# fpthink/PDGN

Measured on AMD Instinct MI355X. Metric: generator+D step points/sec (B=35, 256->2048 pts), higher is better.
Workload: dtype f32; 1 GPU; PDGNet_v2 G+D iteration (models/PDGNet_v2.py:171-256), chair-shaped synthetic batch, per-GPU batch 35, 256->2048 pts, random-init weights; global_batch=35, parallelism=dp1, losses_finite=True, hipgraph=False, issue=list

## Files before the change

include/pdgn_hip.h:

```cpp
#ifndef PDGN_HIP_H
#define PDGN_HIP_H

#include <stdint.h>

#ifdef __cplusplus
extern "C" {
#endif

#define PDGN_ERR_INVALID (-1)
#define PDGN_KNN_MAX_NSAMPLE 200

typedef void *pdgn_stream_t;

#define PDGN_ABI_VERSION 41
int pdgn_abi_version(void);

int pdgn_knnquery(int b, int n, int m, int nsample, const float *xyz, const float *new_xyz,
                  int32_t *idx, float *dist2, pdgn_stream_t stream);

int pdgn_grouping_forward(int b, int c, int n, int m, int nsample, const float *points,
                          const int32_t *idx, float *out, pdgn_stream_t stream);

int pdgn_grouping_backward(int b, int c, int n, int m, int nsample, const float *grad_out,
                           const int32_t *idx, float *grad_points, pdgn_stream_t stream);

int pdgn_nearestneighbor(int b, int n, int m, const float *unknown, const float *known,
                         float *dist2, int32_t *idx, pdgn_stream_t stream);

int pdgn_interpolation_forward(int b, int c, int m, int n, const float *points,
                               const int32_t *idx, const float *weight, float *out,
                               pdgn_stream_t stream);

int pdgn_interpolation_backward(int b, int c, int n, int m, const float *grad_out,
                                const int32_t *idx, const float *weight, float *grad_points,
                                pdgn_stream_t stream);

int pdgn_nndistance(int b, int n, const float *xyz, int m, const float *xyz2, float *result,
                    int32_t *result_i, float *result2, int32_t *result2_i, pdgn_stream_t stream);

int pdgn_nndistance_grad(int b, int n, const float *xyz1, int m, const float *xyz2,
                         const float *grad_dist1, const int32_t *idx1, const float *grad_dist2,
                         const int32_t *idx2, float *grad_xyz1, float *grad_xyz2,
                         pdgn_stream_t stream);

int pdgn_approxmatch(int b, int n, int m, const float *xyz1, const float *xyz2, float *match,
                     float *temp, pdgn_stream_t stream);

int pdgn_matchcost(int b, int n, int m, const float *xyz1, const float *xyz2,
                   const float *match, float *out, pdgn_stream_t stream);

int pdgn_matchcost_grad(int b, int n, int m, const float *xyz1, const float *xyz2,
                        const float *match, float *grad1, float *grad2, pdgn_stream_t stream);

long long pdgn_emd_cost_temp_floats(long long pairs, int n, int m);
int pdgn_emd_cost(int b, int n, int m, const float *xyz1, const float *xyz2, float *temp,
                  float *out, pdgn_stream_t stream);

int pdgn_feature_knn(int b, int f, int n, int k, const float *x, float *sqnorm, int32_t *idx,
                     pdgn_stream_t stream);

int pdgn_window_gather_sum(int b, int n, int k, int ldy, int T, int P, int C, int off, int offc,
                           const float *Y, const int32_t *idx, const float *bias, int bias_bstride,
                           float *out, pdgn_stream_t stream);
int pdgn_window_gather_sum_stats(int b, int n, int k, int ldy, int T, int P, int C, int off, int offc,
                                 const float *Y, const int32_t *idx, const float *bias, int bias_bstride,
                                 float *out, float *scratch, pdgn_stream_t stream);

int pdgn_window_gather_sum_backward(int b, int n, int k, int ldy, int T, int P, int C, int off,
                                    int offc, const float *dout, const int32_t *idx, float *dY,
                                    pdgn_stream_t stream);

int pdgn_knn_graph_transpose(int b, int n, int k, const int32_t *idx, int32_t *rowptr, int32_t *edges,
                             int32_t *scratch, pdgn_stream_t stream);
int pdgn_window_gather_sum_backward_csr(int b, int n, int k, int ldy, int T, int P, int C, int off,
                                        int offc, const float *dout, const int32_t *rowptr,
                                        const int32_t *edges, float *dY, unsigned *max_out, int max_init, pdgn_stream_t stream);

long long pdgn_bn_scratch_floats(long long rows, int c);
int pdgn_bn_stats(long long rows, int c, float eps, float momentum, const float *x, const float *gamma,
                  const float *beta, const float *pre_bias, float *running_mean, float *running_var,
                  float *scratch, float *stats, pdgn_stream_t stream);
int pdgn_bn_eval_stats(int c, float eps, const float *gamma, const float *beta, const float *pre_bias,
                       const float *running_mean, const float *running_var, float *stats,
                       pdgn_stream_t stream);
int pdgn_bn_stats_from_partials(long long rows, int c, float eps, float momentum, const float *gamma,
                                const float *beta, const float *pre_bias, float *running_mean, float *running_var,
                                const float *scratch, float *stats, pdgn_stream_t stream);
int pdgn_bn_stats_from_gemm_partials(long long rows, int c, long long nparts, int block_rows, float eps, float momentum,
                                     const float *gamma, const float *beta, const float *pre_bias,
                                     float *running_mean, float *running_var, const float *partials,
                                     float *stats, double *scratch, pdgn_stream_t stream);
long long pdgn_bn_blocks_scratch_doubles(int c, long long nparts);
int pdgn_bn_act_forward(long long rows, int c, int act, const float *x, const float *stats,
                        const float *mul, float *y, int interleave_n, pdgn_stream_t stream);
int pdgn_bn_act_backward(long long rows, int c, int act, int training, const float *x,
                         const float *dy, const float *mul, const float *stats, float *scratch,
                         float *bsums, float *dx, float *dmul, int interleave_n, pdgn_stream_t stream);

long long pdgn_bn_maxpool_scratch_floats(int b, int c);
int pdgn_bn_act_maxpool(int b, int n, int c, int act, const float *x, const float *stats, float *scratch,
                        float *ymax, int32_t *yarg, pdgn_stream_t stream);
long long pdgn_bn_stats_maxpool_scratch_floats(int b, int c);
int pdgn_bn_stats_act_maxpool(int b, int n, int c, int act, float eps, float momentum, const float *x, const float *gamma,
                              const float *beta, const float *pre_bias, float *running_mean, float *running_var, float *scratch,
                              float *stats, float *ymax, int32_t *yarg, pdgn_stream_t stream);
int pdgn_bn_act_maxpool_backward(int b, int n, int c, int act, int training, const float *x,
                                 const float *dout, const int32_t *yarg, const float *stats,
                                 float *scratch, float *bsums, float *dx, pdgn_stream_t stream);
long long pdgn_dense_bn_maxpool_backward_scratch(int b, int c, int k);
int pdgn_dense_bn_maxpool_backward(int b, int n, int c, int k, int act, const float *x, const float *dout, const int32_t *yarg,
                                   const float *stats, const float *h, int ldh, const float *W, int ldw, float *scratch,
                                   float *dh, float *dW, int lddw, float *bsums, pdgn_stream_t stream);
long long pdgn_dense_bn_maxpool_input_grad_scratch(int b, int c, int k);
int pdgn_dense_bn_maxpool_input_grad(int b, int n, int c, int k, int act, const float *x, const float *dout,
                                     const int32_t *yarg, const float *stats, const float *h, int ldh,
                                     const float *W, int ldw, float *scratch, float *dh, pdgn_stream_t stream);

int pdgn_group_colsum(long long groups, long long group_rows, int c, const float *x, long long ldx, float *out,
                      pdgn_stream_t stream);

int pdgn_softmax_slots_permute(long long m, int k, int c, const float *h, float *w, pdgn_stream_t stream);
int pdgn_bn_softmax_slots_permute(long long m, int k, int c, int act, const float *x, const float *stats,
                                  float *w, pdgn_stream_t stream);
int pdgn_bn_softmax_slots_permute_mul(long long m, int k, int c, int act, const float *x, const float *stats,
                                      int act_u, const float *u, const float *stats_u, float *w, float *y,
                                      unsigned *max_out, const float *gamma_u, const float *beta_u, float bound_scale,
                                      unsigned *cmax_out, pdgn_stream_t stream);
long long pdgn_bilateral_scratch_floats(long long m, int k, int c);
int pdgn_bilateral_weighting_backward(long long m, int k, int c, int act, int training, const float *x,
                                      const float *stats_x, const float *u, const float *stats_u, const float *w,
                                      const float *dy, float *scratch, float *bsums_x, float *bsums_u, float *dx,
                                      float *du, pdgn_stream_t stream);
int pdgn_softmax_slots_permute_backward(long long m, int k, int c, const float *w, const float *dw,
                                        float *dh, pdgn_stream_t stream);

int pdgn_skinny_nt(int R, int N, int K, const float *A, int lda, const float *B, int ldb, const float *bias, float *C, int ldc,
                   pdgn_stream_t stream);
int pdgn_skinny_nn(int R, int N, int K, const float *A, int lda, const float *B, int ldb, float *C, int ldc, pdgn_stream_t stream);
int pdgn_skinny_nt_act(int R, int N, int K, const float *A, int lda, const float *B, int ldb, const float *bias, float *C, int ldc,
                       int act, pdgn_stream_t stream);
int pdgn_skinny_nn_masked(int R, int N, int K, const float *A, int lda, const float *P, int ldp, int act, const float *B,
                          int ldb, float *C, int ldc, pdgn_stream_t stream);
int pdgn_skinny_tn(int R, int N, int K, const float *A, int lda, const float *B, int ldb, float *C, int ldc, pdgn_stream_t stream);
int pdgn_split_bf16x3(int rows, int cols, const float *src, int ld_src, unsigned short *planes, int ld_planes,
                      long long plane_stride, unsigned short *planes_t, int ld_planes_t, long long plane_stride_t,
                      pdgn_stream_t stream);
int pdgn_gemm_nt_ps(long long m, int n, int k, const float *A, int lda, const unsigned short *Wplanes, int ldw, long long wplane,
                    int parts, const float *bias, const float *addend, int ldadd, float *C, int ldc, float *stat_part,
                    const float *row_bias, int ld_rb, int rows_per_group, int act, const float *gate, int ldgate,
                    pdgn_stream_t stream);
long long pdgn_gemm_tail_workspace_floats(long long m, int n, int k, int with_stats);
long long pdgn_gemm_tn_big_workspace_floats(long long m, int n, int k);
int pdgn_gemm_set_tail_workspace(float *ws, long long floats);
int pdgn_gemm_nt_ps_launch_info(long long m, int n, int k, int parts, const void **sym, int *grid);
int pdgn_gemm_aux_symbols(const void **reduce, const void **scan);
int pdgn_gemm_set_mode(int mode);
int pdgn_gemm_set_scale_slots(void *slots, long long bytes);
int pdgn_absmax_rows_cols(long long rows, int cols, const float *src, int ld, unsigned *rowmax, unsigned *colmax,
                          pdgn_stream_t stream);
int pdgn_gemm_set_operand_scales(const unsigned *max_a, const unsigned *max_w);
int pdgn_gemm_two_part(long long m, int n, int k, long long scan_bytes);
int pdgn_gemm_two_part_planes(long long m, int n, int k, long long scan_bytes);
long long pdgn_gemm_nt_ps_stat_rows(long long m, int n, int k, int parts, int plain);
int pdgn_gemm_nt_ps_stat_block_rows(long long m, int n, int k, int parts, int plain);
int pdgn_gemm_nt_ps_row_panel(long long m, int n, int k, int parts, int plain);
long long pdgn_gemm_nt_ps_workspace_floats(long long m, int n, int k, int parts, int with_stats);
int pdgn_split_f16x2(int rows, int cols, const float *src, int ld_src, unsigned short *planes, int ld_planes,
                     long long plane_stride, unsigned short *planes_t, int ld_planes_t, long long plane_stride_t,
                     pdgn_stream_t stream);
int pdgn_gemm_set_config(int cfg);
int pdgn_gemm_set_shape(int shape);
int pdgn_gemm_nt(long long m, int n, int k, const float *A, int lda, const float *W, int ldw,
                 const float *bias, const float *addend, int ldadd, float *C, int ldc, float *stat_part,
                 pdgn_stream_t stream);
long long pdgn_thin_stat_rows(long long m);
int pdgn_thin_stat_block_rows(void);
int pdgn_thin_nt(long long m, int n, int k, const float *X, int ldx, const float *W, int wrs, int wcs,
                 const float *bias, float *Y, int ldy, float *stat_part, pdgn_stream_t stream);
int pdgn_thin_nt_ex(long long m, int n, int k, const float *X, int ldx, const float *W, int wrs, int wcs,
                    const float *bias, float *Y, int ldy, float *stat_part, const float *gate, int ldgate, pdgn_stream_t stream);
int pdgn_thin_tn(long long m, int ta, int wb, const float *A, int lda, const float *B, int ldb, float *O, int osi,
                 int osj, float *sum_a, float *sum_b, pdgn_stream_t stream);
int pdgn_gemm_nn(long long m, int n, int k, const float *A, int lda, const float *Wt, int ldw,
                 const float *bias, const float *addend, int ldadd, float *C, int ldc, float *stat_part,
                 pdgn_stream_t stream);
int pdgn_gemm_tn_big(long long m, int n, int k, const float *dY, int ldy, const float *X, int ldx, float *dW, int dw_is_zero,
                     pdgn_stream_t stream);
int pdgn_gemm_nt_ex(long long m, int n, int k, const float *A, int lda, const float *W, int ldw, const float *bias,
                    const float *addend, int ldadd, float *C, int ldc, float *stat_part, const float *row_bias, int ld_rb,
                    int rows_per_group, int act, const float *gate, int ldgate, int transposed_w, pdgn_stream_t stream);
long long pdgn_gemm_nt_stat_rows(long long m, int n, int k);
int pdgn_gemm_nt_stat_block_rows(long long m, int n, int k);
int pdgn_gemm_nt_config(long long m, int n, int k, int with_stats);

int pdgn_gemm_tn(long long m, int n, int k, const float *dY, const float *X, float *dW,
                 pdgn_stream_t stream);

int pdgn_local_stats(int b, int n, int m, int k, const float *xyz, const int32_t *idx, float *mu,
                     float *cov, pdgn_stream_t stream);
int pdgn_local_stats_backward(int b, int n, int m, int k, const float *xyz, const int32_t *idx,
                              const float *dmu, const float *dcov, float *dxyz, pdgn_stream_t stream);

int pdgn_chamfer_gram(int b, int m, int n, int d, const float *x, const float *y, float *minx,
                      int32_t *argx, float *miny, int32_t *argy, pdgn_stream_t stream);
int pdgn_chamfer_gram_grad(int b, int m, int n, int d, const float *x, const float *y,
                           const float *gminx, const int32_t *argx, const float *gminy,
                           const int32_t *argy, float *gx, float *gy, pdgn_stream_t stream);
int pdgn_chamfer_gram_grad_uniform(int b, int m, int n, int d, const float *x, const float *y, const float *g,
                                   float scale, const int32_t *argx, const int32_t *argy, float *gx, float *gy,
                                   pdgn_stream_t stream);
int pdgn_scaled_sum(long long n, const float *x, float scale, float *out, pdgn_stream_t stream);
int pdgn_mse_const(long long n, const float *x, float target, float scale, float *out, pdgn_stream_t stream);
int pdgn_mse_const_count(long long n, const float *x, float target, float scale, float boundary, float *out, int32_t *count,
                         pdgn_stream_t stream);
int pdgn_mse_const_backward(long long n, const float *x, float target, float scale, const float *g, float *dx,
                            pdgn_stream_t stream);
#define PDGN_GAN_HINGE 1
#define PDGN_GAN_LOGISTIC 2
#define PDGN_GAN_D_REAL 0
#define PDGN_GAN_D_FAKE 1
#define PDGN_GAN_G 2
int pdgn_gan_term(long long n, const float *x, int kind, int role, float scale, float *out, pdgn_stream_t stream);
int pdgn_gan_term_count(long long n, const float *x, int kind, int role, float scale, float boundary, float *out, int32_t *count,
                        pdgn_stream_t stream);
int pdgn_gan_term_backward(long long n, const float *x, int kind, int role, float scale, const float *g, float *dx,
                           pdgn_stream_t stream);

int pdgn_emd_cost_indexed(int npairs, int n, int m, const float *xyz1, const int32_t *ia,
                          const float *xyz2, const int32_t *ib, float *temp, float *out,
                          pdgn_stream_t stream);
int pdgn_chamfer_gram_indexed(int npairs, int m, int n, int d, const float *x, const int32_t *ia,
                              const float *y, const int32_t *ib, float *minx, int32_t *argx,
                              float *miny, int32_t *argy, pdgn_stream_t stream);

int pdgn_deconv_assemble(int F, int Fo, int k, int T, int fc, const float *Wi, const float *W2, const float *Wf,
                         float *WcatC, float *WcatV, float *Wb, pdgn_stream_t stream);
int pdgn_deconv_assemble_backward(int F, int Fo, int k, int T, int fc, const float *gWcatC, const float *gWcatV,
                                  const float *gWb, float *dWi, float *dW2, float *dWf, pdgn_stream_t stream);

int pdgn_sample_bias(int b, int ldy, int nspec, const int *T, const int *C, const int *off, const int *offc,
                     const float *const *bias, const float *Yc, float *bb, pdgn_stream_t stream);
int pdgn_sample_bias_backward(int b, int ldy, int nspec, const int *T, const int *C, const int *off, const int *offc,
                              const float *g, float *dYc, float *const *dbias, pdgn_stream_t stream);

int pdgn_small_mlp_forward(int r, int k, int n, int act, int bn_mode, float eps, float momentum, const float *x,
                           const float *W, const float *bias, const float *gamma, const float *beta,
                           float *running_mean, float *running_var, float *y, float *pre, float *stat,
                           pdgn_stream_t stream);
int pdgn_small_mlp_backward(int r, int k, int n, int act, int bn_mode, const float *x, const float *dy, const float *pre,
                            const float *stat, const float *gamma, const float *beta, float *dpre, float *dgamma,
                            float *dbeta, float *dbias, float *dW, pdgn_stream_t stream);

int pdgn_ballquery(int b, int n, int m, float radius, int nsample, const float *new_xyz, const float *xyz,
                   int32_t *idx, pdgn_stream_t stream);
int pdgn_furthestsampling(int b, int n, int m, const float *xyz, float *temp, int32_t *idx, pdgn_stream_t stream);
int pdgn_gathering_forward(int b, int c, int n, int m, const float *points, const int32_t *idx, float *out,
                           pdgn_stream_t stream);
int pdgn_gathering_backward(int b, int c, int n, int m, const float *grad_out, const int32_t *idx,
                            float *grad_points, pdgn_stream_t stream);
int pdgn_grouping_int_forward(int b, int c, int n, int m, int nsample, const long long *points, const int32_t *idx,
                              long long *out, pdgn_stream_t stream);
int pdgn_featuredistribute(int b, int n, int m, const float *max_xyz, const float *xyz, int32_t *distribute_idx,
                           pdgn_stream_t stream);
int pdgn_labelstat_idx(int b, int n, int m, int nsample, int nclass, const int32_t *label_stat, const int32_t *idx,
                       int32_t *new_label_stat, pdgn_stream_t stream);
int pdgn_labelstat_ballrange(int b, int n, int m, float radius, int nclass, const float *new_xyz, const float *xyz,
                             const int32_t *label_stat, int32_t *new_label_stat, pdgn_stream_t stream);
int pdgn_labelstat_and_ballquery(int b, int n, int m, float radius, int nsample, int nclass, const float *new_xyz,
                                 const float *xyz, const int32_t *label_stat, int32_t *idx, int32_t *new_label_stat,
                                 pdgn_stream_t stream);

long long pdgn_point_max_scratch(int b, int n, int c);
int pdgn_point_max(int b, int n, int c, const float *x, float *scratch_val, int32_t *scratch_arg, float *out, int32_t *arg,
                   pdgn_stream_t stream);
int pdgn_point_max_backward(int b, int n, int c, const float *grad_out, const int32_t *arg, float *grad_x,
                            pdgn_stream_t stream);

int pdgn_spin(unsigned int microseconds, pdgn_stream_t stream);

int pdgn_replay_marker(int id, pdgn_stream_t stream);
int pdgn_replay_build(void *hip_graph, void **plan_out);
int pdgn_replay_info(void *plan, int *counts8);
int pdgn_replay_chains(void *plan, int *labels, int *nodes_per_chain);
int pdgn_replay_set_stream(void *plan, int chain, pdgn_stream_t stream);
int pdgn_replay_launch(void *plan);
int pdgn_replay_launch_range(void *plan, int lo, int hi);
int pdgn_replay_position(void *plan, int chain, int nth);
int pdgn_replay_points(void *plan, int *ids, int *pos, int *chain, int max_out);
int pdgn_replay_joined(void *plan);
int pdgn_replay_kernel_nodes(void *plan, const void *sym, int gx, int *pos, int max_out);
int pdgn_replay_chain_neighbor(void *plan, int pos, int dir, int *kind_out, const void **sym_out);
int pdgn_replay_time_spans(void *plan, const int *first, const int *last, int n, int slots);
int pdgn_replay_time_read(void *plan, float *ms_out, int *counts);
int pdgn_replay_launch_timed(void *plan, double *us32);
int pdgn_replay_probe_chain(void *plan, int chain, int stride, float *ms_out, int *pos_out, int max_out);
int pdgn_replay_destroy(void *plan);

int pdgn_adam_multi(int ntensors, void *const *p, const void *const *g, void *const *m, void *const *v, const long long *n, double lr,
                    double beta1, double beta2, double eps, const float *step, pdgn_stream_t stream);
int pdgn_copy_multi(int ntensors, void *const *dst, const void *const *src, const long long *n, pdgn_stream_t stream);
int pdgn_adam_ema_multi(int ntensors, void *const *p, const void *const *g, void *const *m, void *const *v, void *const *e,
                        const long long *n, double lr, double beta1, double beta2, double eps, double ema_decay, const float *step,
                        pdgn_stream_t stream);
int pdgn_ema_multi(int ntensors, void *const *e, const void *const *p, const long long *n, double ema_decay, const float *step,
                   pdgn_stream_t stream);

typedef struct pdgn_guard_record {
    float norm;
    float coef;
    float applied;
    float found_inf;
    unsigned n_applied;
    unsigned n_skipped;
    unsigned reserved[2];
} pdgn_guard_record;
long long pdgn_gradnorm_workspace_doubles(int ntensors, const long long *n);
int pdgn_gradnorm_multi(int ntensors, const void *const *g, const long long *n, double max_norm, double *workspace,
                        long long workspace_doubles, pdgn_guard_record *record, pdgn_stream_t stream);
int pdgn_adam_guard_multi(int ntensors, void *const *p, const void *const *g, void *const *m, void *const *v, const long long *n,
                          double lr, double beta1, double beta2, double eps, const float *step, const pdgn_guard_record *guard,
                          pdgn_stream_t stream);
int pdgn_adam_ema_guard_multi(int ntensors, void *const *p, const void *const *g, void *const *m, void *const *v, void *const *e,
                              const long long *n, double lr, double beta1, double beta2, double eps, double ema_decay, const float *step,
                              const pdgn_guard_record *guard, pdgn_stream_t stream);
int pdgn_ema_guard_multi(int ntensors, void *const *e, const void *const *p, const long long *n, double ema_decay, const float *step,
                         const pdgn_guard_record *guard, pdgn_stream_t stream);

#define PDGN_LR_MAX_KNOTS 16
#define PDGN_LR_TABLE_DOUBLES 33
int pdgn_adam_sched_multi(int ntensors, void *const *p, const void *const *g, void *const *m, void *const *v, void *const *e,
                          const long long *n, double lr, double beta1, double beta2, double eps, double ema_decay, const float *step,
                          const pdgn_guard_record *guard, const double *sched, pdgn_stream_t stream);
int pdgn_lr_eval(const double *sched, double lr, const float *step, const pdgn_guard_record *guard, double *out2, float *out_lr32,
                 pdgn_stream_t stream);

int pdgn_set_deterministic(int on);
long long pdgn_det_workspace_ints(int b, int targets, long long edges);
int pdgn_grouping_backward_det(int b, int c, int n, int m, int nsample, const float *grad_out, const int32_t *idx,
                               int32_t *ws, float *grad_points, pdgn_stream_t stream);
int pdgn_interpolation_backward_det(int b, int c, int n, int m, const float *grad_out, const int32_t *idx,
                                    const float *weight, int32_t *ws, float *grad_points, pdgn_stream_t stream);
int pdgn_gathering_backward_det(int b, int c, int n, int m, const float *grad_out, const int32_t *idx, int32_t *ws,
                                float *grad_points, pdgn_stream_t stream);
int pdgn_nndistance_grad_det(int b, int n, const float *xyz1, int m, const float *xyz2, const float *grad_dist1,
                             const int32_t *idx1, const float *grad_dist2, const int32_t *idx2, int32_t *ws,
                             float *grad_xyz1, float *grad_xyz2, pdgn_stream_t stream);

int pdgn_feed_batch(int B, int S, int N, int r1, int r2, int r3, const float *data, const int32_t *order, long long first,
                    unsigned long long seed, unsigned long long t, long long row0, float sigma, float *p1, float *p2, float *p3,
                    float *p4, float *z1, float *z2, pdgn_stream_t stream);

int pdgn_feed_batch_resample(int B, int S, int M, int P, int N, int r1, int r2, int r3, const float *data, const int32_t *order,
                             long long first, unsigned long long seed, unsigned long long t, long long row0, float sigma, float *p1,
                             float *p2, float *p3, float *p4, float *z1, float *z2, pdgn_stream_t stream);

int pdgn_feed_batch_mesh(int B, int S, int V, int F, int N, int r1, int r2, int r3, const float *verts, const int32_t *faces,
                         const int32_t *face_off, const uint32_t *alias, const int32_t *order, long long first, unsigned long long seed,
                         unsigned long long t, long long row0, float sigma, float *p1, float *p2, float *p3, float *p4, float *z1,
                         float *z2, int32_t *face_rec, pdgn_stream_t stream);

int pdgn_sample_surface(int S, int n, const float *verts, const int32_t *faces, const int32_t *face_off, const uint32_t *alias,
                        unsigned long long seed, unsigned long long draw, float *out, int32_t *face_rec, pdgn_stream_t stream);

int pdgn_feed_batch_ragged(int B, int S, int N, int r1, int r2, int r3, const float *points, const long long *off, long long T,
                           const int32_t *order, long long first, unsigned long long seed, unsigned long long t, long long row0,
                           float sigma, float *p1, float *p2, float *p3, float *p4, float *z1, float *z2, pdgn_stream_t stream);

int pdgn_sample_ragged(int S, int n, const float *points, const long long *off, long long T, unsigned long long seed,
                       unsigned long long draw, float *out , pdgn_stream_t stream);

#define PDGN_FPS_MAX_N 8192
int pdgn_fps_order(int b, int n, int m, const float *xyz, const int32_t *start, int32_t *order, pdgn_stream_t stream);

#define PDGN_FEED_TAG_FPS 7
int pdgn_feed_fps_pyramid(int B, int N, int r1, int r2, int r3, const float *p4, unsigned long long seed, unsigned long long t,
                          long long row0, float *p1, float *p2, float *p3, int32_t *order_out, pdgn_stream_t stream);

typedef struct pdgn_aug_table {
    unsigned thr_flip, thr_rot, thr_scale, thr_trans, thr_jitter;
    int flip_axis, up_axis;
    float rot_max;
    float log_scale_max;
    float trans_max;
    float sigma;
    unsigned reserved[5];
} pdgn_aug_table;
#define PDGN_AUG_TAG_BASE 16
#define PDGN_AUG_SITES 12
int pdgn_augment_rows_fwd(int B, int N, const float *x, int x_point_major, float *rows, float *affine_out, const pdgn_aug_table *table,
                          const unsigned long long *clock, unsigned long long seed, long long row0, int tag, pdgn_stream_t stream);
int pdgn_augment_rows_bwd(int B, int N, const float *d_rows, float *dx, int dx_point_major, const pdgn_aug_table *table,
                          const unsigned long long *clock, unsigned long long seed, long long row0, int tag, pdgn_stream_t stream);
int pdgn_augment_tick(unsigned long long *clock, pdgn_stream_t stream);

typedef struct pdgn_ada_state {
    double target;
    unsigned long long interval;
    unsigned long long span;
    unsigned long long thr_min, thr_max;
    unsigned long long mask;
// ... 42 lines not shown
```

pdgn_amd/csrc/bnact.hip:

```cpp
#include "common.h"

#include "bn_geom.h"
#define ACT_NONE 0
#define ACT_RELU 1
#define ACT_LEAKY 2

__device__ __forceinline__ float act_fwd(float z, int act) {
    if (act == ACT_RELU) return fmaxf(z, 0.f);
    if (act == ACT_LEAKY) return z > 0.f ? z : 0.01f * z;
    return z;
}
__device__ __forceinline__ float act_grad(float z, int act) {
    if (act == ACT_RELU) return z > 0.f ? 1.f : 0.f;
    if (act == ACT_LEAKY) return z > 0.f ? 1.f : 0.01f;
    return 1.f;
}

struct ClGeom {
    int cg, cgb, rl;
};

__global__ __launch_bounds__(BN_THREADS) void cl_stats_kernel(long long R, int C, int cgb, int rows_per_block,
                                                              const float *__restrict__ x,
                                                              float *__restrict__ part) {
    __shared__ float4 red[2][BN_THREADS];
    const int cgl = threadIdx.x % cgb, rlane = threadIdx.x / cgb, rl = BN_THREADS / cgb;
    const int cgi = blockIdx.x * cgb + cgl;
    const bool cok = cgi * 4 < C;
    const long long r0 = (long long)blockIdx.y * rows_per_block;
    const long long r1 = min(R, r0 + rows_per_block);
    float4 s = make_float4(0.f, 0.f, 0.f, 0.f), q = make_float4(0.f, 0.f, 0.f, 0.f);
    if (cok) {
        const float *X = x + cgi * 4;
        const float4 pv = *reinterpret_cast<const float4 *>(X);
        long long r = r0 + rlane;
        for (; r + 3LL * rl < r1; r += 4LL * rl) {
            float4 v[4];
#pragma unroll
            for (int u = 0; u < 4; ++u) v[u] = *reinterpret_cast<const float4 *>(X + (r + (long long)u * rl) * C);
#pragma unroll
            for (int u = 0; u < 4; ++u) {
                const float dx = v[u].x - pv.x, dy = v[u].y - pv.y, dz = v[u].z - pv.z, dw = v[u].w - pv.w;
                s.x += dx; s.y += dy; s.z += dz; s.w += dw;
                q.x = __fmaf_rn(dx, dx, q.x); q.y = __fmaf_rn(dy, dy, q.y);
                q.z = __fmaf_rn(dz, dz, q.z); q.w = __fmaf_rn(dw, dw, q.w);
            }
        }
        for (; r < r1; r += rl) {
            const float4 v = *reinterpret_cast<const float4 *>(X + r * C);
            const float dx = v.x - pv.x, dy = v.y - pv.y, dz = v.z - pv.z, dw = v.w - pv.w;
            s.x += dx; s.y += dy; s.z += dz; s.w += dw;
            q.x = __fmaf_rn(dx, dx, q.x); q.y = __fmaf_rn(dy, dy, q.y);
            q.z = __fmaf_rn(dz, dz, q.z); q.w = __fmaf_rn(dw, dw, q.w);
        }
    }
    red[0][threadIdx.x] = s;
    red[1][threadIdx.x] = q;
    __syncthreads();
    if (rlane == 0 && cok) {
        for (int j = 1; j < rl; ++j) {
            float4 a = red[0][j * cgb + cgl], b = red[1][j * cgb + cgl];
            s.x += a.x; s.y += a.y; s.z += a.z; s.w += a.w;
            q.x += b.x; q.y += b.y; q.z += b.z; q.w += b.w;
        }
        float *P = part + (size_t)blockIdx.y * 2 * C;
        *reinterpret_cast<float4 *>(P + cgi * 4) = s;
        *reinterpret_cast<float4 *>(P + C + cgi * 4) = q;
    }
}

#define FIN_CH 4
#define FIN_PL 64

__device__ __forceinline__ double fin_reduce(const float *__restrict__ part, int nparts, size_t ld, int c, bool ok,
                                             double (*red)[FIN_CH]) {
    const int cl = threadIdx.x % FIN_CH, pl = threadIdx.x / FIN_CH;
    double s = 0;
    if (ok) {
        int p = pl;
        for (; p + 3 * FIN_PL < nparts; p += 4 * FIN_PL) {
            const float a0 = part[(size_t)p * ld + c], a1 = part[(size_t)(p + FIN_PL) * ld + c];
            const float a2 = part[(size_t)(p + 2 * FIN_PL) * ld + c], a3 = part[(size_t)(p + 3 * FIN_PL) * ld + c];
            s += ((double)a0 + (double)a1) + ((double)a2 + (double)a3);
        }
        for (; p < nparts; p += FIN_PL) s += (double)part[(size_t)p * ld + c];
    }
    red[pl][cl] = s;
    __syncthreads();
    for (int h = FIN_PL / 2; h > 0; h >>= 1) {
        if (pl < h) red[pl][cl] += red[pl + h][cl];
        __syncthreads();
    }
    return red[0][cl];
}

__device__ __forceinline__ void fin_reduce2(const float *__restrict__ part, int nparts, size_t ld, int c, int C, bool ok,
                                            double (*red)[FIN_CH], double (*red2)[FIN_CH], double &s1, double &s2) {
    const int cl = threadIdx.x % FIN_CH, pl = threadIdx.x / FIN_CH;
    double a = 0, b = 0;
    if (ok) {
        int p = pl;
        for (; p + 3 * FIN_PL < nparts; p += 4 * FIN_PL) {
            const float *q = part + (size_t)p * ld + c;
            const float a0 = q[0], a1 = q[(size_t)FIN_PL * ld], a2 = q[(size_t)2 * FIN_PL * ld], a3 = q[(size_t)3 * FIN_PL * ld];
            const float b0 = q[C], b1 = q[(size_t)FIN_PL * ld + C], b2 = q[(size_t)2 * FIN_PL * ld + C], b3 = q[(size_t)3 * FIN_PL * ld + C];
            a += ((double)a0 + (double)a1) + ((double)a2 + (double)a3);
            b += ((double)b0 + (double)b1) + ((double)b2 + (double)b3);
        }
        for (; p < nparts; p += FIN_PL) {
            a += (double)part[(size_t)p * ld + c];
            b += (double)part[(size_t)p * ld + C + c];
        }
    }
    red[pl][cl] = a;
    red2[pl][cl] = b;
    __syncthreads();
    for (int h = FIN_PL / 2; h > 0; h >>= 1) {
        if (pl < h) {
            red[pl][cl] += red[pl + h][cl];
            red2[pl][cl] += red2[pl + h][cl];
        }
        __syncthreads();
    }
    s1 = red[0][cl];
    s2 = red2[0][cl];
}

__global__ __launch_bounds__(FIN_CH * FIN_PL) void cl_finalize_kernel(
    long long R, int C, int nparts, float eps, float momentum, const float *__restrict__ part,
    const float *__restrict__ gamma, const float *__restrict__ beta, const float *__restrict__ pre_bias,
    float *__restrict__ running_mean, float *__restrict__ running_var, float *__restrict__ stats,
    const float *__restrict__ pivot) {
    __shared__ double red[FIN_PL][FIN_CH], red2[FIN_PL][FIN_CH];
    const int c = blockIdx.x * FIN_CH + threadIdx.x % FIN_CH;
    const bool ok = c < C;
    double s1, s2;
    fin_reduce2(part, nparts, (size_t)2 * C, c, C, ok, red, red2, s1, s2);
    if (!ok || threadIdx.x >= FIN_CH) return;
    const double ms = s1 / (double)R;
    double var = s2 / (double)R - ms * ms;
    var = var < 0 ? 0 : var;
    const double mean = ms + (pivot ? (double)pivot[c] : 0.0);
    const float invstd = (float)(1.0 / sqrt(var + (double)eps));
    const float g = gamma ? gamma[c] : 1.f, b = beta ? beta[c] : 0.f;
    const float scale = g * invstd;
    stats[c] = scale;
    stats[C + c] = b - (float)mean * scale;
    stats[2 * C + c] = (float)mean;
    stats[3 * C + c] = invstd;
    if (running_mean) {
        const double unbiased = R > 1 ? var * (double)R / (double)(R - 1) : var;
        const float mb = (float)mean + (pre_bias ? pre_bias[c] : 0.f);
        running_mean[c] = (1.f - momentum) * running_mean[c] + momentum * mb;
        running_var[c] = (1.f - momentum) * running_var[c] + momentum * (float)unbiased;
    }
}

__global__ __launch_bounds__(FIN_CH * FIN_PL) void cl_finalize_blocks_kernel(
    long long R, int C, int nparts, int rpp, float eps, float momentum, const float *__restrict__ part,
    const float *__restrict__ gamma, const float *__restrict__ beta, const float *__restrict__ pre_bias,
    float *__restrict__ running_mean, float *__restrict__ running_var, float *__restrict__ stats) {
    __shared__ double red[FIN_PL][FIN_CH], red2[FIN_PL][FIN_CH];
    const int cl = threadIdx.x % FIN_CH, pl = threadIdx.x / FIN_CH;
    const int c = blockIdx.x * FIN_CH + cl;
    const bool ok = c < C;
    double a = 0, b = 0;
    const double inv_full = 1.0 / (double)rpp;
    const int pmax = (int)min((long long)nparts, (R + rpp - 1) / rpp);
    if (ok)
#pragma unroll 4
        for (int p = pl; p < pmax; p += FIN_PL) {
            const long long left = R - (long long)p * rpp;
            const bool full = left >= rpp;
            const double n = (double)(full ? rpp : left), inv = full ? inv_full : 1.0 / (double)left;
            const float *q = part + (size_t)p * 3 * C + c;
            const double s = (double)q[0], sq = (double)q[C], pv = (double)q[2 * C];
            const double mb = pv + s * inv;
            a += n * mb;
            b += (sq - s * s * inv) + n * mb * mb;
        }
    red[pl][cl] = a;
    red2[pl][cl] = b;
    __syncthreads();
    for (int h = FIN_PL / 2; h > 0; h >>= 1) {
        if (pl < h) {
            red[pl][cl] += red[pl + h][cl];
            red2[pl][cl] += red2[pl + h][cl];
        }
        __syncthreads();
    }
    if (!ok || threadIdx.x >= FIN_CH) return;
    const double mean = red[0][cl] / (double)R;
    double var = red2[0][cl] / (double)R - mean * mean;
    var = var < 0 ? 0 : var;
    const float invstd = (float)(1.0 / sqrt(var + (double)eps));
    const float g = gamma ? gamma[c] : 1.f, be = beta ? beta[c] : 0.f;
    const float scale = g * invstd;
    stats[c] = scale;
    stats[C + c] = be - (float)mean * scale;
    stats[2 * C + c] = (float)mean;
    stats[3 * C + c] = invstd;
    if (running_mean) {
        const double unbiased = R > 1 ? var * (double)R / (double)(R - 1) : var;
        const float mb = (float)mean + (pre_bias ? pre_bias[c] : 0.f);
        running_mean[c] = (1.f - momentum) * running_mean[c] + momentum * mb;
        running_var[c] = (1.f - momentum) * running_var[c] + momentum * (float)unbiased;
    }
}

__global__ __launch_bounds__(FIN_CH * FIN_PL) void cl_finalize_blocks_slice_kernel(
    long long R, int C, int nparts, int rpp, int per_slice, const float *__restrict__ part, double *__restrict__ scratch) {
    __shared__ double red[FIN_PL][FIN_CH], red2[FIN_PL][FIN_CH];
    const int cl = threadIdx.x % FIN_CH, pl = threadIdx.x / FIN_CH;
    const int c = blockIdx.x * FIN_CH + cl;
    const bool ok = c < C;
    double a = 0, b = 0;
    const double inv_full = 1.0 / (double)rpp;
    const int pmax_all = (int)min((long long)nparts, (R + rpp - 1) / rpp);
    const int p0 = blockIdx.y * per_slice, pmax = min(pmax_all, p0 + per_slice);
    if (ok)
#pragma unroll 4
        for (int p = p0 + pl; p < pmax; p += FIN_PL) {
            const long long left = R - (long long)p * rpp;
            const bool full = left >= rpp;
            const double n = (double)(full ? rpp : left), inv = full ? inv_full : 1.0 / (double)left;
            const float *q = part + (size_t)p * 3 * C + c;
            const double s = (double)q[0], sq = (double)q[C], pv = (double)q[2 * C];
            const double mb = pv + s * inv;
            a += n * mb;
            b += (sq - s * s * inv) + n * mb * mb;
        }
    red[pl][cl] = a;
    red2[pl][cl] = b;
    __syncthreads();
    for (int h = FIN_PL / 2; h > 0; h >>= 1) {
        if (pl < h) {
            red[pl][cl] += red[pl + h][cl];
            red2[pl][cl] += red2[pl + h][cl];
        }
        __syncthreads();
    }
    if (!ok || threadIdx.x >= FIN_CH) return;
    scratch[((size_t)blockIdx.y * 2) * C + c] = red[0][cl];
    scratch[((size_t)blockIdx.y * 2 + 1) * C + c] = red2[0][cl];
}

__global__ __launch_bounds__(256) void cl_finalize_blocks_slice64_kernel(
    long long R, int C, int nparts, int rpp, int per_slice, const float *__restrict__ part, double *__restrict__ scratch) {
    __shared__ double red[4][64], red2[4][64];
    const int cl = threadIdx.x & 63, pl = threadIdx.x >> 6;
    const int c = blockIdx.x * 64 + cl;
    double a = 0, b = 0;
    const double inv_full = 1.0 / (double)rpp;
    const int pmax_all = (int)min((long long)nparts, (R + rpp - 1) / rpp);
    const int p0 = blockIdx.y * per_slice, pmax = min(pmax_all, p0 + per_slice);
#pragma unroll 4
    for (int p = p0 + pl; p < pmax; p += 4) {
        const long long left = R - (long long)p * rpp;
        const bool full = left >= rpp;
        const double n = (double)(full ? rpp : left), inv = full ? inv_full : 1.0 / (double)left;
        const float *q = part + (size_t)p * 3 * C + c;
        const double s = (double)q[0], sq = (double)q[C], pv = (double)q[2 * C];
        const double mb = pv + s * inv;
        a += n * mb;
        b += (sq - s * s * inv) + n * mb * mb;
    }
    red[pl][cl] = a;
    red2[pl][cl] = b;
    __syncthreads();
    if (pl == 0) {
        scratch[((size_t)blockIdx.y * 2) * C + c] = ((red[0][cl] + red[1][cl]) + red[2][cl]) + red[3][cl];
        scratch[((size_t)blockIdx.y * 2 + 1) * C + c] = ((red2[0][cl] + red2[1][cl]) + red2[2][cl]) + red2[3][cl];
    }
}

__global__ void cl_finalize_blocks_join_kernel(long long R, int C, int slices, float eps, float momentum,
                                               const double *__restrict__ scratch, const float *__restrict__ gamma,
                                               const float *__restrict__ beta, const float *__restrict__ pre_bias,
                                               float *__restrict__ running_mean, float *__restrict__ running_var,
                                               float *__restrict__ stats) {
    __shared__ double ra[4][64], rb[4][64];
    const int cl = threadIdx.x & 63, pl = threadIdx.x >> 6;
    const int c = blockIdx.x * 64 + cl;
    double a = 0, b = 0;
    if (c < C)
        for (int s = pl; s < slices; s += 4) {
            a += scratch[((size_t)s * 2) * C + c];
            b += scratch[((size_t)s * 2 + 1) * C + c];
        }
    ra[pl][cl] = a;
    rb[pl][cl] = b;
    __syncthreads();
    if (pl != 0 || c >= C) return;
    a = ((ra[0][cl] + ra[1][cl]) + ra[2][cl]) + ra[3][cl];
    b = ((rb[0][cl] + rb[1][cl]) + rb[2][cl]) + rb[3][cl];
    const double mean = a / (double)R;
    double var = b / (double)R - mean * mean;
    var = var < 0 ? 0 : var;
    const float invstd = (float)(1.0 / sqrt(var + (double)eps));
    const float g = gamma ? gamma[c] : 1.f, be = beta ? beta[c] : 0.f;
    const float scale = g * invstd;
    stats[c] = scale;
    stats[C + c] = be - (float)mean * scale;
    stats[2 * C + c] = (float)mean;
    stats[3 * C + c] = invstd;
    if (running_mean) {
        const double unbiased = R > 1 ? var * (double)R / (double)(R - 1) : var;
        const float mb = (float)mean + (pre_bias ? pre_bias[c] : 0.f);
        running_mean[c] = (1.f - momentum) * running_mean[c] + momentum * mb;
        running_var[c] = (1.f - momentum) * running_var[c] + momentum * (float)unbiased;
    }
}

static inline int fb_slices(int c, long long nparts) {
    if (nparts < 512) return 0;
    if (c % 64 == 0) {
        if (nparts <= 1400) return 0;
        long long s64 = nparts / 64;
        return (int)(s64 < 2 ? 2 : (s64 > 128 ? 128 : s64));
    }
    long long s = 512 / (c / 4 > 0 ? c / 4 : 1);
    s = s > 32 ? 32 : s;
    while (s > 1 && nparts / s < 128) s >>= 1;
    return s < 2 ? 0 : (int)s;
}

__global__ void cl_eval_stats_kernel(int C, float eps, const float *__restrict__ gamma, const float *__restrict__ beta,
                                     const float *__restrict__ pre_bias, const float *__restrict__ running_mean,
                                     const float *__restrict__ running_var, float *__restrict__ stats) {
    const int c = blockIdx.x * blockDim.x + threadIdx.x;
    if (c >= C) return;
    const float invstd = rsqrtf(running_var[c] + eps);
    const float g = gamma ? gamma[c] : 1.f, b = beta ? beta[c] : 0.f;
    const float m = running_mean[c] - (pre_bias ? pre_bias[c] : 0.f);
    stats[c] = g * invstd;
    stats[C + c] = b - m * g * invstd;
    stats[2 * C + c] = m;
    stats[3 * C + c] = invstd;
}

__device__ __forceinline__ void cl_interleaved_rows(long long r, int pn, long long &ra, long long &rb) {
    const long long b = r / pn;
    ra = b * 2 * pn + (r - b * pn);
    rb = ra + pn;
}

__global__ __launch_bounds__(BN_THREADS) void cl_apply_kernel(long long R, int C, int cgb, int rows_per_block, int act,
                                                              const float *__restrict__ x,
                                                              const float *__restrict__ stats,
                                                              const float *__restrict__ mul, float *__restrict__ y, int pn) {
    const int cgl = threadIdx.x % cgb, rlane = threadIdx.x / cgb, rl = BN_THREADS / cgb;
    const int cgi = blockIdx.x * cgb + cgl;
    if (cgi * 4 >= C) return;
    const long long r0 = (long long)blockIdx.y * rows_per_block;
    const long long r1 = min(R, r0 + rows_per_block);
    const float4 sc = *reinterpret_cast<const float4 *>(stats + cgi * 4);
    const float4 sh = *reinterpret_cast<const float4 *>(stats + C + cgi * 4);
    const bool has_mul = mul != nullptr;
    for (long long r = r0 + rlane; r < r1; r += 4 * rl) {
        float4 v[4], m[4];
#pragma unroll
        for (int u = 0; u < 4; ++u) {
            const long long rr = r + (long long)u * rl;
            if (rr < r1) {
                v[u] = *reinterpret_cast<const float4 *>(x + rr * C + cgi * 4);
                if (has_mul) m[u] = *reinterpret_cast<const float4 *>(mul + rr * C + cgi * 4);
            }
        }
#pragma unroll
        for (int u = 0; u < 4; ++u) {
            const long long rr = r + (long long)u * rl;
            if (rr < r1) {
                float4 o;
                o.x = act_fwd(__fmaf_rn(v[u].x, sc.x, sh.x), act); o.y = act_fwd(__fmaf_rn(v[u].y, sc.y, sh.y), act);
                o.z = act_fwd(__fmaf_rn(v[u].z, sc.z, sh.z), act); o.w = act_fwd(__fmaf_rn(v[u].w, sc.w, sh.w), act);
                if (has_mul) { o.x *= m[u].x; o.y *= m[u].y; o.z *= m[u].z; o.w *= m[u].w; }
                if (pn) {
                    long long ra, rb;
                    cl_interleaved_rows(rr, pn, ra, rb);
                    *reinterpret_cast<float2 *>(y + ra * (C / 2) + cgi * 2) = make_float2(o.x, o.z);
                    *reinterpret_cast<float2 *>(y + rb * (C / 2) + cgi * 2) = make_float2(o.y, o.w);
                } else {
                    *reinterpret_cast<float4 *>(y + rr * C + cgi * 4) = o;
                }
            }
        }
    }
}

__global__ __launch_bounds__(BN_THREADS) void cl_bwd_reduce_kernel(long long R, int C, int cgb, int rows_per_block,
                                                                   int act, const float *__restrict__ x,
                                                                   const float *__restrict__ dy,
                                                                   const float *__restrict__ mul,
                                                                   const float *__restrict__ stats,
                                                                   float *__restrict__ part, int pn) {
    __shared__ float4 red[2][BN_THREADS];
    const int cgl = threadIdx.x % cgb, rlane = threadIdx.x / cgb, rl = BN_THREADS / cgb;
    const int cgi = blockIdx.x * cgb + cgl;
    const bool cok = cgi * 4 < C;
    const long long r0 = (long long)blockIdx.y * rows_per_block;
    const long long r1 = min(R, r0 + rows_per_block);
    float4 s = make_float4(0.f, 0.f, 0.f, 0.f), q = make_float4(0.f, 0.f, 0.f, 0.f);
    if (cok) {
        const float4 sc = *reinterpret_cast<const float4 *>(stats + cgi * 4);
        const float4 sh = *reinterpret_cast<const float4 *>(stats + C + cgi * 4);
        const float4 mu = *reinterpret_cast<const float4 *>(stats + 2 * C + cgi * 4);
        const float4 is = *reinterpret_cast<const float4 *>(stats + 3 * C + cgi * 4);
        const bool has_mul = mul != nullptr;
        for (long long rb = r0 + rlane; rb < r1; rb += 4LL * rl) {
            float4 v[4], g[4], m[4];
#pragma unroll
            for (int u = 0; u < 4; ++u) {
                const long long r = rb + (long long)u * rl;
                if (r < r1) {
                    v[u] = *reinterpret_cast<const float4 *>(x + r * C + cgi * 4);
                    if (pn) {
                        long long ra, rbb;
                        cl_interleaved_rows(r, pn, ra, rbb);
                        const float2 ga = *reinterpret_cast<const float2 *>(dy + ra * (C / 2) + cgi * 2);
                        const float2 gb = *reinterpret_cast<const float2 *>(dy + rbb * (C / 2) + cgi * 2);
                        g[u] = make_float4(ga.x, gb.x, ga.y, gb.y);
                    } else {
                        g[u] = *reinterpret_cast<const float4 *>(dy + r * C + cgi * 4);
                    }
                    if (has_mul) m[u] = *reinterpret_cast<const float4 *>(mul + r * C + cgi * 4);
                }
            }
#pragma unroll
            for (int u = 0; u < 4; ++u) {
                if (rb + (long long)u * rl < r1) {
                    if (has_mul) { g[u].x *= m[u].x; g[u].y *= m[u].y; g[u].z *= m[u].z; g[u].w *= m[u].w; }
                    float dz;
                    dz = g[u].x * act_grad(__fmaf_rn(v[u].x, sc.x, sh.x), act); s.x += dz; q.x = __fmaf_rn(dz, (v[u].x - mu.x) * is.x, q.x);
                    dz = g[u].y * act_grad(__fmaf_rn(v[u].y, sc.y, sh.y), act); s.y += dz; q.y = __fmaf_rn(dz, (v[u].y - mu.y) * is.y, q.y);
                    dz = g[u].z * act_grad(__fmaf_rn(v[u].z, sc.z, sh.z), act); s.z += dz; q.z = __fmaf_rn(dz, (v[u].z - mu.z) * is.z, q.z);
                    dz = g[u].w * act_grad(__fmaf_rn(v[u].w, sc.w, sh.w), act); s.w += dz; q.w = __fmaf_rn(dz, (v[u].w - mu.w) * is.w, q.w);
                }
            }
        }
    }
    red[0][threadIdx.x] = s;
    red[1][threadIdx.x] = q;
    __syncthreads();
    if (rlane == 0 && cok) {
        for (int j = 1; j < rl; ++j) {
            float4 a = red[0][j * cgb + cgl], b = red[1][j * cgb + cgl];
            s.x += a.x; s.y += a.y; s.z += a.z; s.w += a.w;
            q.x += b.x; q.y += b.y; q.z += b.z; q.w += b.w;
        }
        float *P = part + (size_t)blockIdx.y * 2 * C;
        *reinterpret_cast<float4 *>(P + cgi * 4) = s;
        *reinterpret_cast<float4 *>(P + C + cgi * 4) = q;
    }
}

__global__ __launch_bounds__(FIN_CH * FIN_PL) void cl_bwd_finalize_kernel(long long R, int C, int nparts, int training,
                                                                         const float *__restrict__ part,
                                                                         const float *__restrict__ stats,
                                                                         float *__restrict__ bsums,
                                                                         float *__restrict__ coef) {
    __shared__ double red[FIN_PL][FIN_CH], red2[FIN_PL][FIN_CH];
    const int c = blockIdx.x * FIN_CH + threadIdx.x % FIN_CH;
    const bool ok = c < C;
    double s1, s2;
    fin_reduce2(part, nparts, (size_t)2 * C, c, C, ok, red, red2, s1, s2);
    if (!ok || threadIdx.x >= FIN_CH) return;
    bsums[c] = (float)s1;
    bsums[C + c] = (float)s2;
    float ca = 0.f, cb = 0.f;
    if (training) {
        const float sc = stats[c], mu = stats[2 * C + c], is = stats[3 * C + c];
        cb = sc * is * (float)(s2 / (double)R);
        ca = sc * (float)(s1 / (double)R) - cb * mu;
    }
    coef[c] = ca;
    coef[C + c] = cb;
}

__global__ __launch_bounds__(BN_THREADS) void cl_bwd_apply_kernel(long long R, int C, int cgb, int rows_per_block, int act,
                                                                  const float *__restrict__ x,
                                                                  const float *__restrict__ dy,
                                                                  const float *__restrict__ mul,
                                                                  const float *__restrict__ stats,
                                                                  const float *__restrict__ coef,
                                                                  float *__restrict__ dx, float *__restrict__ dmul, int pn) {
    const int cgl = threadIdx.x % cgb, rlane = threadIdx.x / cgb, rl = BN_THREADS / cgb;
    const int cgi = blockIdx.x * cgb + cgl;
    if (cgi * 4 >= C) return;
    const long long r0 = (long long)blockIdx.y * rows_per_block;
    const long long r1 = min(R, r0 + rows_per_block);
    float sc[4], sh[4], ca[4], cb[4];
    *reinterpret_cast<float4 *>(sc) = *reinterpret_cast<const float4 *>(stats + cgi * 4);
    *reinterpret_cast<float4 *>(sh) = *reinterpret_cast<const float4 *>(stats + C + cgi * 4);
    *reinterpret_cast<float4 *>(ca) = *reinterpret_cast<const float4 *>(coef + cgi * 4);
    *reinterpret_cast<float4 *>(cb) = *reinterpret_cast<const float4 *>(coef + C + cgi * 4);
    const bool has_mul = mul != nullptr, want_dmul = dmul != nullptr;
    for (long long r = r0 + rlane; r < r1; r += 4 * rl) {
        float v[4][4], g[4][4], m[4][4];
#pragma unroll
        for (int u = 0; u < 4; ++u) {
            const long long rr = r + (long long)u * rl;
            if (rr < r1) {
                *reinterpret_cast<float4 *>(v[u]) = *reinterpret_cast<const float4 *>(x + rr * C + cgi * 4);
                if (pn) {
                    long long ra, rb;
                    cl_interleaved_rows(rr, pn, ra, rb);
                    const float2 ga = *reinterpret_cast<const float2 *>(dy + ra * (C / 2) + cgi * 2);
                    const float2 gb = *reinterpret_cast<const float2 *>(dy + rb * (C / 2) + cgi * 2);
                    g[u][0] = ga.x; g[u][1] = gb.x; g[u][2] = ga.y; g[u][3] = gb.y;
                } else {
                    *reinterpret_cast<float4 *>(g[u]) = *reinterpret_cast<const float4 *>(dy + rr * C + cgi * 4);
                }
                if (has_mul) *reinterpret_cast<float4 *>(m[u]) = *reinterpret_cast<const float4 *>(mul + rr * C + cgi * 4);
            }
        }
#pragma unroll
        for (int u = 0; u < 4; ++u) {
            const long long rr = r + (long long)u * rl;
            if (rr < r1) {
                float o[4], om[4];
#pragma unroll
                for (int j = 0; j < 4; ++j) {
                    const float z = __fmaf_rn(v[u][j], sc[j], sh[j]);
                    om[j] = g[u][j] * act_fwd(z, act);
                    const float dz = (has_mul ? g[u][j] * m[u][j] : g[u][j]) * act_grad(z, act);
                    o[j] = __fmaf_rn(sc[j], dz, -ca[j]) - cb[j] * v[u][j];
                }
                *reinterpret_cast<float4 *>(dx + rr * C + cgi * 4) = *reinterpret_cast<float4 *>(o);
                if (want_dmul) *reinterpret_cast<float4 *>(dmul + rr * C + cgi * 4) = *reinterpret_cast<float4 *>(om);
            }
        }
    }
}

extern "C" long long pdgn_bn_scratch_floats(long long rows, int c) {
    if (rows < 1 || c < 4 || c % 4) return PDGN_ERR_INVALID;
    int cgb, gx, gy, rpb;
    cl_geometry(rows, c, &cgb, &gx, &gy, &rpb);
    return (long long)gy * 2 * c + 2 * c;
}

extern "C" int pdgn_bn_stats(long long rows, int c, float eps, float momentum, const float *x, const float *gamma,
                             const float *beta, const float *pre_bias, float *running_mean, float *running_var,
                             float *scratch, float *stats, pdgn_stream_t stream) {
    if (rows < 1 || c < 4 || c % 4) return PDGN_ERR_INVALID;
    hipStream_t s = (hipStream_t)stream;
    int cgb, gx, gy, rpb;
    cl_geometry(rows, c, &cgb, &gx, &gy, &rpb);
    hipLaunchKernelGGL(cl_stats_kernel, dim3(gx, gy), dim3(BN_THREADS), 0, s, rows, c, cgb, rpb, x, scratch);
    hipLaunchKernelGGL(cl_finalize_kernel, dim3(cdiv(c, FIN_CH)), dim3(FIN_CH * FIN_PL), 0, s, rows, c, gy, eps, momentum, scratch,
                       gamma, beta, pre_bias, running_mean, running_var, stats, x);
    return pdgn_launch_status();
}

extern "C" int pdgn_bn_stats_from_partials(long long rows, int c, float eps, float momentum, const float *gamma,
                                           const float *beta, const float *pre_bias, float *running_mean,
                                           float *running_var, const float *scratch, float *stats, pdgn_stream_t stream) {
    if (rows < 1 || c < 4 || c % 4) return PDGN_ERR_INVALID;
    int cgb, gx, gy, rpb;
    cl_geometry(rows, c, &cgb, &gx, &gy, &rpb);
    hipLaunchKernelGGL(cl_finalize_kernel, dim3(cdiv(c, FIN_CH)), dim3(FIN_CH * FIN_PL), 0, (hipStream_t)stream, rows, c, gy, eps,
                       momentum, scratch, gamma, beta, pre_bias, running_mean, running_var, stats, (const float *)nullptr);
    return pdgn_launch_status();
}

extern "C" int pdgn_bn_stats_from_gemm_partials(long long rows, int c, long long nparts, int block_rows, float eps,
                                                float momentum, const float *gamma, const float *beta, const float *pre_bias,
                                                float *running_mean, float *running_var, const float *partials,
                                                float *stats, double *scratch, pdgn_stream_t stream) {
    if (rows < 1 || c < 4 || c % 4 || nparts < 1 || nparts > 0x7fffffffLL || block_rows < 1 ||
        nparts * (long long)block_rows < rows)
        return PDGN_ERR_INVALID;
    const int slices = scratch ? fb_slices(c, nparts) : 0;
    if (slices > 1) {
        const int per = (int)((nparts + slices - 1) / slices);
        if (c % 64 == 0)
            hipLaunchKernelGGL(cl_finalize_blocks_slice64_kernel, dim3(c / 64, slices), dim3(256), 0, (hipStream_t)stream, rows, c, (int)nparts,
                               block_rows, per, partials, scratch);
        else
            hipLaunchKernelGGL(cl_finalize_blocks_slice_kernel, dim3(cdiv(c, FIN_CH), slices), dim3(FIN_CH * FIN_PL), 0,
                               (hipStream_t)stream, rows, c, (int)nparts, block_rows, per, partials, scratch);
        hipLaunchKernelGGL(cl_finalize_blocks_join_kernel, dim3(cdiv(c, 64)), dim3(256), 0, (hipStream_t)stream, rows, c, slices,
                           eps, momentum, (const double *)scratch, gamma, beta, pre_bias, running_mean, running_var, stats);
        return pdgn_launch_status();
    }
    hipLaunchKernelGGL(cl_finalize_blocks_kernel, dim3(cdiv(c, FIN_CH)), dim3(FIN_CH * FIN_PL), 0, (hipStream_t)stream, rows, c,
                       (int)nparts, block_rows, eps, momentum, partials, gamma, beta, pre_bias, running_mean, running_var, stats);
    return pdgn_launch_status();
}

extern "C" long long pdgn_bn_blocks_scratch_doubles(int c, long long nparts) {
    if (c < 1 || nparts < 1) return PDGN_ERR_INVALID;
    return (long long)fb_slices(c, nparts) * 2 * c;
}

extern "C" int pdgn_bn_eval_stats(int c, float eps, const float *gamma, const float *beta, const float *pre_bias,
                                  const float *running_mean, const float *running_var, float *stats,
                                  pdgn_stream_t stream) {
    if (c < 1) return PDGN_ERR_INVALID;
    hipLaunchKernelGGL(cl_eval_stats_kernel, dim3(cdiv(c, 256)), dim3(256), 0, (hipStream_t)stream, c, eps, gamma,
                       beta, pre_bias, running_mean, running_var, stats);
    return pdgn_launch_status();
}

extern "C" int pdgn_bn_act_forward(long long rows, int c, int act, const float *x, const float *stats, const float *mul,
                                   float *y, int interleave_n, pdgn_stream_t stream) {
    if (rows < 1 || c < 4 || c % 4 || act < 0 || act > 2) return PDGN_ERR_INVALID;
    if (interleave_n < 0 || (interleave_n > 0 && (rows % interleave_n || mul))) return PDGN_ERR_INVALID;
    int cgb, gx, gy, rpb;
    cl_geometry(rows, c, &cgb, &gx, &gy, &rpb);
    hipLaunchKernelGGL(cl_apply_kernel, dim3(gx, gy), dim3(BN_THREADS), 0, (hipStream_t)stream, rows, c, cgb, rpb, act,
                       x, stats, mul, y, interleave_n);
    return pdgn_launch_status();
}

extern "C" int pdgn_bn_act_backward(long long rows, int c, int act, int training, const float *x, const float *dy,
                                    const float *mul, const float *stats, float *scratch, float *bsums, float *dx,
                                    float *dmul, int interleave_n, pdgn_stream_t stream) {
    if (rows < 1 || c < 4 || c % 4 || act < 0 || act > 2) return PDGN_ERR_INVALID;
    if (interleave_n < 0 || (interleave_n > 0 && (rows % interleave_n || mul))) return PDGN_ERR_INVALID;
    hipStream_t s = (hipStream_t)stream;
    int cgb, gx, gy, rpb;
    cl_geometry(rows, c, &cgb, &gx, &gy, &rpb);
    hipLaunchKernelGGL(cl_bwd_reduce_kernel, dim3(gx, gy), dim3(BN_THREADS), 0, s, rows, c, cgb, rpb, act, x, dy, mul,
                       stats, scratch, interleave_n);
    float *coef = scratch + (size_t)gy * 2 * c;
    hipLaunchKernelGGL(cl_bwd_finalize_kernel, dim3(cdiv(c, FIN_CH)), dim3(FIN_CH * FIN_PL), 0, s, rows, c, gy, training,
                       scratch, stats, bsums, coef);
    hipLaunchKernelGGL(cl_bwd_apply_kernel, dim3(gx, gy), dim3(BN_THREADS), 0, s, rows, c, cgb, rpb, act, x, dy, mul,
                       stats, coef, dx, dmul, interleave_n);
    return pdgn_launch_status();
}

#define BW_MAXK 16

template <int KT, bool APPLY>
__global__ __launch_bounds__(BN_THREADS) void bilateral_bwd_kernel(
    long long M, int k_rt, int C, int cpb, int m_per_block, int act, const float *__restrict__ x,
    const float *__restrict__ stats_x, const float *__restrict__ u, const float *__restrict__ stats_u,
    const float *__restrict__ w, const float *__restrict__ dy, float *__restrict__ part_x, float *__restrict__ part_u,
    const float *__restrict__ coef_x, const float *__restrict__ coef_u, float *__restrict__ dx, float *__restrict__ du) {
    constexpr int KM = KT ? KT : BW_MAXK;
    __shared__ float red[12][BN_THREADS];
    const int k = KT ? KT : k_rt, P = k / 2, C2 = C / 2, Cu = 2 * C;
    const int cpl = threadIdx.x % cpb, rlane = threadIdx.x / cpb, rl = BN_THREADS / cpb;
    const int cp = blockIdx.x * cpb + cpl;
    const bool ok = cp < C2;
    const int c = 2 * (ok ? cp : 0);
    const long long m0 = (long long)blockIdx.y * m_per_block, m1 = min(M, m0 + m_per_block);
    const float2 scx = *reinterpret_cast<const float2 *>(stats_x + c), shx = *reinterpret_cast<const float2 *>(stats_x + C + c);
    const float2 mux = *reinterpret_cast<const float2 *>(stats_x + 2 * C + c), isx = *reinterpret_cast<const float2 *>(stats_x + 3 * C + c);
    const float4 scu = *reinterpret_cast<const float4 *>(stats_u + 2 * c), shu = *reinterpret_cast<const float4 *>(stats_u + Cu + 2 * c);
    const float4 muu = *reinterpret_cast<const float4 *>(stats_u + 2 * Cu + 2 * c), isu = *reinterpret_cast<const float4 *>(stats_u + 3 * Cu + 2 * c);
    float2 cax = make_float2(0.f, 0.f), cbx = cax;
    float4 cau = make_float4(0.f, 0.f, 0.f, 0.f), cbu = cau;
    if (APPLY) {
        cax = *reinterpret_cast<const float2 *>(coef_x + c); cbx = *reinterpret_cast<const float2 *>(coef_x + C + c);
        cau = *reinterpret_cast<const float4 *>(coef_u + 2 * c); cbu = *reinterpret_cast<const float4 *>(coef_u + Cu + 2 * c);
    }
    float acc[12];
#pragma unroll
    for (int i = 0; i < 12; ++i) acc[i] = 0.f;
    if (ok)
        for (long long m = m0 + rlane; m < m1; m += rl) {
            const size_t ox = (size_t)m * k * C + c, ou = (size_t)m * k * C + 2 * c;
            float2 xv[KM];
            float4 uv[KM / 2], wv[KM / 2], gv[KM / 2];
#pragma unroll
            for (int s = 0; s < KM; ++s)
                if (KT || s < k) xv[s] = *reinterpret_cast<const float2 *>(x + ox + (size_t)s * C);
#pragma unroll
            for (int p = 0; p < KM / 2; ++p)
                if (KT || p < P) {
                    uv[p] = *reinterpret_cast<const float4 *>(u + ou + (size_t)p * Cu);
                    if (w) wv[p] = *reinterpret_cast<const float4 *>(w + ou + (size_t)p * Cu);
                    gv[p] = *reinterpret_cast<const float4 *>(dy + ou + (size_t)p * Cu);
                }
            if (!w) {
                float h0[KM], h1[KM];
                float mx0 = -INFINITY, mx1 = -INFINITY;
#pragma unroll
                for (int s = 0; s < KM; ++s)
                    if (KT || s < k) {
                        h0[s] = act_fwd(__fmaf_rn(xv[s].x, scx.x, shx.x), act);
                        h1[s] = act_fwd(__fmaf_rn(xv[s].y, scx.y, shx.y), act);
                        mx0 = fmaxf(mx0, h0[s]);
                        mx1 = fmaxf(mx1, h1[s]);
                    }
                float e0 = 0.f, e1 = 0.f;
#pragma unroll
                for (int s = 0; s < KM; ++s)
                    if (KT || s < k) {
                        h0[s] = __expf(h0[s] - mx0);
                        h1[s] = __expf(h1[s] - mx1);
                        e0 += h0[s];
                        e1 += h1[s];
                    }
                const float i0 = 1.0f / e0, i1 = 1.0f / e1;
#pragma unroll
                for (int p = 0; p < KM / 2; ++p)
                    if (KT || p < P) wv[p] = make_float4(h0[p] * i0, h0[P + p] * i0, h1[p] * i1, h1[P + p] * i1);
            }
            float dot0 = 0.f, dot1 = 0.f;
#pragma unroll
            for (int p = 0; p < KM / 2; ++p)
                if (KT || p < P) {
                    const float u4[4] = {uv[p].x, uv[p].y, uv[p].z, uv[p].w}, w4[4] = {wv[p].x, wv[p].y, wv[p].z, wv[p].w};
                    const float g4[4] = {gv[p].x, gv[p].y, gv[p].z, gv[p].w};
                    const float s4[4] = {scu.x, scu.y, scu.z, scu.w}, h4[4] = {shu.x, shu.y, shu.z, shu.w};
                    const float m4[4] = {muu.x, muu.y, muu.z, muu.w}, i4[4] = {isu.x, isu.y, isu.z, isu.w};
                    const float a4[4] = {cau.x, cau.y, cau.z, cau.w}, b4[4] = {cbu.x, cbu.y, cbu.z, cbu.w};
                    float dW[4], o4[4];
#pragma unroll
                    for (int j = 0; j < 4; ++j) {
                        const float z = __fmaf_rn(u4[j], s4[j], h4[j]);
                        dW[j] = g4[j] * act_fwd(z, act);
                        const float dz = g4[j] * w4[j] * act_grad(z, act);
                        if (APPLY) o4[j] = __fmaf_rn(s4[j], dz, -a4[j]) - b4[j] * u4[j];
                        else { acc[4 + j] += dz; acc[8 + j] = __fmaf_rn(dz, (u4[j] - m4[j]) * i4[j], acc[8 + j]); }
                    }
                    if (APPLY) *reinterpret_cast<float4 *>(du + ou + (size_t)p * Cu) = make_float4(o4[0], o4[1], o4[2], o4[3]);
                    dot0 = __fmaf_rn(w4[0], dW[0], __fmaf_rn(w4[1], dW[1], dot0));
                    dot1 = __fmaf_rn(w4[2], dW[2], __fmaf_rn(w4[3], dW[3], dot1));
                    gv[p] = make_float4(dW[0], dW[1], dW[2], dW[3]);
                }
#pragma unroll
            for (int s = 0; s < KM; ++s)
                if (KT || s < k) {
                    const int p = s < P ? s : s - P;
                    const bool hi = s >= P;
                    const float w0 = hi ? wv[p].y : wv[p].x, g0 = hi ? gv[p].y : gv[p].x;
                    const float w1 = hi ? wv[p].w : wv[p].z, g1 = hi ? gv[p].w : gv[p].z;
                    const float da0 = w0 * (g0 - dot0), da1 = w1 * (g1 - dot1);
                    const float dz0 = da0 * act_grad(__fmaf_rn(xv[s].x, scx.x, shx.x), act);
                    const float dz1 = da1 * act_grad(__fmaf_rn(xv[s].y, scx.y, shx.y), act);
                    if (APPLY) {
                        float2 o;
                        o.x = __fmaf_rn(scx.x, dz0, -cax.x) - cbx.x * xv[s].x;
                        o.y = __fmaf_rn(scx.y, dz1, -cax.y) - cbx.y * xv[s].y;
                        *reinterpret_cast<float2 *>(dx + ox + (size_t)s * C) = o;
                    } else {
                        acc[0] += dz0; acc[1] += dz1;
                        acc[2] = __fmaf_rn(dz0, (xv[s].x - mux.x) * isx.x, acc[2]);
                        acc[3] = __fmaf_rn(dz1, (xv[s].y - mux.y) * isx.y, acc[3]);
                    }
                }
        }
    if (APPLY) return;
#pragma unroll
    for (int i = 0; i < 12; ++i) red[i][threadIdx.x] = acc[i];
    __syncthreads();
    if (rlane == 0 && ok) {
        for (int j = 1; j < rl; ++j)
#pragma unroll
            for (int i = 0; i < 12; ++i) acc[i] += red[i][j * cpb + cpl];
        float *px = part_x + (size_t)blockIdx.y * 2 * C, *pu = part_u + (size_t)blockIdx.y * 2 * Cu;
        *reinterpret_cast<float2 *>(px + c) = make_float2(acc[0], acc[1]);
        *reinterpret_cast<float2 *>(px + C + c) = make_float2(acc[2], acc[3]);
        *reinterpret_cast<float4 *>(pu + 2 * c) = make_float4(acc[4], acc[5], acc[6], acc[7]);
        *reinterpret_cast<float4 *>(pu + Cu + 2 * c) = make_float4(acc[8], acc[9], acc[10], acc[11]);
    }
}

static void bw_geometry(long long M, int C, int *cpb, int *gx, int *gy, int *mpb) {
    const int c2 = C / 2;
    int p = 1;
    while (p < c2 && p < BN_THREADS) p <<= 1;
    *cpb = p;
    *gx = (c2 + p - 1) / p;
    const int rl = BN_THREADS / p;
    long long want = 1024 / *gx;
    want = want < 1 ? 1 : want;
    long long rows = (M + want - 1) / want;
    rows = rows < (long long)rl * 4 ? (long long)rl * 4 : rows;
    rows = rows > 4096 ? 4096 : rows;
    rows = (rows + rl - 1) / rl * rl;
    *mpb = (int)rows;
    *gy = (int)((M + rows - 1) / rows);
}

extern "C" long long pdgn_bilateral_scratch_floats(long long m, int k, int c) {
    if (m < 1 || k < 2 || (k & 1) || k > BW_MAXK || c < 2 || (c & 1)) return PDGN_ERR_INVALID;
    int cpb, gx, gy, mpb;
    bw_geometry(m, c, &cpb, &gx, &gy, &mpb);
    return (long long)gy * 6 * c + 6 * c;
}

extern "C" int pdgn_bilateral_weighting_backward(long long m, int k, int c, int act, int training, const float *x,
                                                 const float *stats_x, const float *u, const float *stats_u,
                                                 const float *w, const float *dy, float *scratch, float *bsums_x,
                                                 float *bsums_u, float *dx, float *du, pdgn_stream_t stream) {
    if (m < 1 || k < 2 || (k & 1) || k > BW_MAXK || c < 4 || (c % 4) || act < 0 || act > 2) return PDGN_ERR_INVALID;
    hipStream_t s = (hipStream_t)stream;
    int cpb, gx, gy, mpb;
    bw_geometry(m, c, &cpb, &gx, &gy, &mpb);
    float *part_x = scratch, *part_u = part_x + (size_t)gy * 2 * c;
    float *coef_x = part_u + (size_t)gy * 4 * c, *coef_u = coef_x + 2 * c;
    const dim3 grid(gx, gy), block(BN_THREADS);
#define BW_LAUNCH(KT, AP)                                                                                              \
    hipLaunchKernelGGL((bilateral_bwd_kernel<KT, AP>), grid, block, 0, s, m, k, c, cpb, mpb, act, x, stats_x, u, stats_u, w, \
                       dy, part_x, part_u, coef_x, coef_u, dx, du)
    if (k == 10) BW_LAUNCH(10, false); else if (k == 4) BW_LAUNCH(4, false); else BW_LAUNCH(0, false);
    hipLaunchKernelGGL(cl_bwd_finalize_kernel, dim3(cdiv(c, FIN_CH)), dim3(FIN_CH * FIN_PL), 0, s, m * k, c, gy, training, part_x,
                       stats_x, bsums_x, coef_x);
    hipLaunchKernelGGL(cl_bwd_finalize_kernel, dim3(cdiv(2 * c, FIN_CH)), dim3(FIN_CH * FIN_PL), 0, s, m * (k / 2), 2 * c, gy,
                       training, part_u, stats_u, bsums_u, coef_u);
    if (k == 10) BW_LAUNCH(10, true); else if (k == 4) BW_LAUNCH(4, true); else BW_LAUNCH(0, true);
#undef BW_LAUNCH
    return pdgn_launch_status();
}

#define MP_SPLIT 16

__global__ __launch_bounds__(BN_THREADS) void cl_apply_max_kernel(int N, int C, int cgb, int act,
                                                                  const float *__restrict__ x,
                                                                  const float *__restrict__ stats,
                                                                  float *__restrict__ pmax, int32_t *__restrict__ parg) {
    __shared__ float smax[BN_THREADS][4];
    __shared__ int sarg[BN_THREADS][4];
    const int cgl = threadIdx.x % cgb, rlane = threadIdx.x / cgb, rl = BN_THREADS / cgb;
    const int cgi = blockIdx.x * cgb + cgl;
    const bool cok = cgi * 4 < C;
    const int b = blockIdx.z, sp = blockIdx.y;
    const int per = (N + MP_SPLIT - 1) / MP_SPLIT;
    const int n0 = sp * per, n1 = min(N, n0 + per);
    float best[4] = {-INFINITY, -INFINITY, -INFINITY, -INFINITY};
    int arg[4] = {n0, n0, n0, n0};
    if (cok) {
        float sc[4], sh[4];
// ... 569 lines not shown
```

pdgn_amd/deconv.py:

```python
import ctypes

import torch
import torch.nn as nn
import torch.nn.functional as F
from ._fn import Function

from . import _lib
from . import streams as _streams
from ._lib import check, ptr, require, stream_of
from .fused import (Planes, split_planes, skinny_linear, _zeros, bilateral_weighting, bn_act,
                    small_sequential, bn_act_maxpool, bn_softmax_slots_permute, flush_bn_counters,
                    has_zero_colsum, linear_cl, softmax_slots_permute, DenseInput, group_colsum, mark_maxima, row_maxima_buffer)
from .fused import _STATS_MAX as STATS_MAX

F32, I32 = torch.float32, torch.int32
_KNN_OVERLAP = __import__("os").environ.get("PDGN_KNN_OVERLAP", "1") == "1"
_KNN_CONST = __import__("os").environ.get("PDGN_KNN_CONST", "0") == "1"

def _knn_stream(device):
    return _streams.plan(device).knn


def _w2d(conv):
    w = conv.weight
    return w.view(w.shape[0], w.shape[1])


KNN_LOG = None


def feature_knn(x, k):
    require(x, "x", F32, 3)
    b, f, n = x.shape
    if KNN_LOG is not None:
        KNN_LOG.append((b, f, n))
    idx = torch.empty((b, n, k), dtype=I32, device=x.device)
    sq = torch.empty((b, n), dtype=F32, device=x.device)
    check(_lib.lib().pdgn_feature_knn(b, f, n, int(k), ptr(x), ptr(sq), ptr(idx), stream_of(x)),
          "pdgn_feature_knn")
    return idx


def start_feature_knn(xt, const, k, x_cf=None):
    want_csr = torch.is_grad_enabled() and xt.requires_grad

    def channel_major():
        if x_cf is not None:
            return x_cf.detach().contiguous()
        x = xt.detach().transpose(1, 2)
        if const is not None and _KNN_CONST:
            x = torch.cat((const.detach().unsqueeze(2).expand(-1, -1, xt.shape[1]), x), 1)
        return x.contiguous()

    with torch.no_grad():
        if not (xt.is_cuda and _KNN_OVERLAP):
            return feature_knn(channel_major(), k), None
        cur = torch.cuda.current_stream(xt.device)
        side = _knn_stream(xt.device)
        side.wait_stream(cur)
        for t in (xt, const, x_cf):
            if t is not None:
                t.record_stream(side)
        with torch.cuda.stream(side):
            x_knn = channel_major()
            idx = feature_knn(x_knn, k)
            ready = torch.cuda.Event()
            ready.record(side)
            if want_csr:
                transposed_graph(idx)
                idx._pdgn_csr_ready = torch.cuda.Event()
                idx._pdgn_csr_ready.record(side)
    return idx, ready


class EdgeGatherSum(Function):

    @staticmethod
    def forward(ctx, Y, idx, specs, *biases):
        require(Y, "Y", F32, 3)
        require(idx, "idx", I32, 3)
        b, n, ldy = Y.shape
        k = idx.shape[2]
        outs, partials = [], []
        L = _lib.lib()
        for spec, bias in zip(specs, biases):
            T, P, C, off, offc = spec[:5]
            out = torch.empty((b, n, P, C), dtype=F32, device=Y.device)
            if bias is not None and bias.dim() == 2 and bias.stride(1) == 1:
                bias_c, bstride = bias.detach(), bias.stride(0)
            else:
                bias_c = bias.detach().contiguous() if bias is not None else None
                bstride = C if (bias is not None and bias.dim() == 2) else 0
            if len(spec) > 5 and spec[5]:
                scr = torch.empty(L.pdgn_bn_scratch_floats(b * n * P, C), dtype=F32, device=Y.device)
                check(L.pdgn_window_gather_sum_stats(b, n, k, ldy, T, P, C, off, offc, ptr(Y), ptr(idx), ptr(bias_c),
                                                     bstride, ptr(out), ptr(scr), stream_of(Y)),
                      "pdgn_window_gather_sum_stats")
                partials.append(scr)
            else:
                check(L.pdgn_window_gather_sum(b, n, k, ldy, T, P, C, off, offc, ptr(Y), ptr(idx),
                                               ptr(bias_c), bstride, ptr(out), stream_of(Y)),
                      "pdgn_window_gather_sum")
            outs.append(out)
        specs = tuple(tuple(spec[:5]) for spec in specs)
        ctx.mark_non_differentiable(*partials)
        ctx.set_materialize_grads(False)
        ctx.specs, ctx.shape = specs, (b, n, ldy, k)
        ctx.has_bias = [0 if bias is None else bias.dim() for bias in biases]
        ctx.save_for_backward(idx)
        return tuple(outs) + tuple(partials)

    @staticmethod
    def backward(ctx, *douts):
        (idx,) = ctx.saved_tensors
        b, n, ldy, k = ctx.shape
        douts = [d if d is not None else torch.zeros((b, n, P, C), dtype=F32, device=idx.device)
                 for d, (T, P, C, off, offc) in zip(douts, ctx.specs)]
        L = _lib.lib()
        covered = sum(T * C + (C if offc >= 0 else 0) for (T, P, C, off, offc) in ctx.specs)
        vec_ok = ldy % 4 == 0 and k <= 31 and all(C % 4 == 0 and off % 4 == 0 and (offc < 0 or offc % 4 == 0)
                                                 for (T, P, C, off, offc) in ctx.specs)
        dbias = []
        if vec_ok and covered == ldy:
            rowptr, edges = transposed_graph(idx)
            dY = torch.empty((b, n, ldy), dtype=F32, device=idx.device)
            dmax = row_maxima_buffer(b * n, idx.device) if (_lib.gemm_mode() == "x2" and b * n * ldy >= (1 << 24)) else None
            first = 1
            for (T, P, C, off, offc), dout, hb in zip(ctx.specs, douts, ctx.has_bias):
                hb = 3 if hb == 1 and has_zero_colsum(dout) else hb
                dout = dout.contiguous()
                check(L.pdgn_window_gather_sum_backward_csr(b, n, k, ldy, T, P, C, off, offc, ptr(dout), ptr(rowptr),
                                                            ptr(edges), ptr(dY), ptr(dmax), first, stream_of(dout)),
                      "pdgn_window_gather_sum_backward_csr")
                first = 0
                if hb == 2 and offc >= 0:
                    dbias.append(group_colsum(dY.view(b * n, ldy)[:, offc:offc + C], n))
                else:
                    dbias.append(_dbias(dout, hb))
            if dmax is not None:
                mark_maxima(dY, dmax)
            return (dY, None, None) + tuple(dbias)
        dY = torch.zeros((b, n, ldy), dtype=F32, device=idx.device)
        for (T, P, C, off, offc), dout, hb in zip(ctx.specs, douts, ctx.has_bias):
            hb = 3 if hb == 1 and has_zero_colsum(dout) else hb
            dout = dout.contiguous()
            check(L.pdgn_window_gather_sum_backward(b, n, k, ldy, T, P, C, off, offc, ptr(dout), ptr(idx), ptr(dY),
                                                    stream_of(dout)), "pdgn_window_gather_sum_backward")
            dbias.append(_dbias(dout, hb))
        return (dY, None, None) + tuple(dbias)


def _dbias(dout, kind):
    if kind == 0:
        return None
    if kind == 3:
        return _zeros((dout.shape[-1],), dout.device)
    C = dout.shape[-1]
    if dout.is_contiguous():
        return group_colsum(dout.view(-1, C))[0] if kind == 1 else group_colsum(dout.view(-1, C), dout.shape[1] * dout.shape[2])
    return dout.sum(dim=(0, 1, 2)) if kind == 1 else dout.sum(dim=(1, 2))


def transposed_graph(idx):
    cached = getattr(idx, "_pdgn_csr", None)
    if cached is not None:
        ev = getattr(idx, "_pdgn_csr_ready", None)
        if ev is not None:
            torch.cuda.current_stream(idx.device).wait_event(ev)
        return cached
    b, n, k = idx.shape
    rowptr = torch.empty((b, n + 1), dtype=I32, device=idx.device)
    edges = torch.empty((b, n * k), dtype=I32, device=idx.device)
    scratch = torch.empty((2 * b * n,), dtype=I32, device=idx.device)
    check(_lib.lib().pdgn_knn_graph_transpose(b, n, k, ptr(idx), ptr(rowptr), ptr(edges), ptr(scratch),
                                              stream_of(idx)), "pdgn_knn_graph_transpose")
    idx._pdgn_csr = (rowptr, edges)
    return idx._pdgn_csr


class SampleBias(Function):

    @staticmethod
    def _arrays(meta):
        n = len(meta)
        mk = lambda j: (ctypes.c_int * n)(*[m[j] for m in meta])
        return n, mk(0), mk(1), mk(2), mk(3)

    @staticmethod
    def forward(ctx, Yc, meta, *biases):
        Yc = Yc.contiguous()
        B, ldy = Yc.shape
        n, T, C, off, offc = SampleBias._arrays(meta)
        bs = [b.detach().contiguous() if b is not None else None for b in biases]
        bp = (ctypes.c_void_p * n)(*[b.data_ptr() if b is not None else None for b in bs])
        bb = torch.empty((B, sum(m[1] for m in meta)), dtype=F32, device=Yc.device)
        check(_lib.lib().pdgn_sample_bias(B, ldy, n, T, C, off, offc, bp, ptr(Yc), ptr(bb), stream_of(Yc)), "pdgn_sample_bias")
        ctx.meta, ctx.shape = meta, (B, ldy)
        ctx.has = [b is not None for b in biases]
        return bb

    @staticmethod
    def backward(ctx, g):
        meta, (B, ldy) = ctx.meta, ctx.shape
        n, T, C, off, offc = SampleBias._arrays(meta)
        g = g.contiguous()
        covered = sum(m[0] * m[1] + m[1] for m in meta)
        dYc = (torch.empty if covered == ldy else torch.zeros)((B, ldy), dtype=F32, device=g.device)
        dbs = [torch.empty(m[1], dtype=F32, device=g.device) if h and ctx.needs_input_grad[2 + i] else None
               for i, (m, h) in enumerate(zip(meta, ctx.has))]
        dp = (ctypes.c_void_p * n)(*[d.data_ptr() if d is not None else None for d in dbs])
        check(_lib.lib().pdgn_sample_bias_backward(B, ldy, n, T, C, off, offc, ptr(g), ptr(dYc), dp, stream_of(g)),
              "pdgn_sample_bias_backward")
        return (dYc, None) + tuple(dbs)


class AssembleWeights(Function):

    @staticmethod
    def forward(ctx, Wi, W2, Wf, F_, Fo, k, T, Fc):
        Wi, W2 = Wi.contiguous(), W2.contiguous()
        Wf = Wf.contiguous() if Wf is not None else None
        P = k - T + 1
        Mw = T * 4 * F_ + 4 * F_ + k * 2 * Fo + 2 * Fo + (32 if Wf is not None else 0)
        dev = Wi.device
        WcatC = torch.empty((Mw, Fc), dtype=F32, device=dev) if Fc else None
        WcatV = torch.empty((Mw, F_ - Fc), dtype=F32, device=dev)
        Wb = torch.empty((2 * Fo, P * 4 * F_), dtype=F32, device=dev)
        check(_lib.lib().pdgn_deconv_assemble(F_, Fo, k, T, Fc, ptr(Wi), ptr(W2), ptr(Wf), ptr(WcatC), ptr(WcatV), ptr(Wb),
                                              stream_of(Wi)), "pdgn_deconv_assemble")
        ctx.cfg = (F_, Fo, k, T, Fc, Wi.shape, W2.shape, None if Wf is None else Wf.shape)
        return WcatC, WcatV, Wb

    @staticmethod
    def backward(ctx, gC, gV, gB):
        F_, Fo, k, T, Fc, si, s2, sf = ctx.cfg
        ref = gV if gV is not None else (gB if gB is not None else gC)
        gC = gC.contiguous() if gC is not None else None
        gV = gV.contiguous() if gV is not None else None
        gB = gB.contiguous() if gB is not None else None
        dWi = torch.empty(si, dtype=F32, device=ref.device)
        dW2 = torch.empty(s2, dtype=F32, device=ref.device)
        dWf = torch.empty(sf, dtype=F32, device=ref.device) if sf is not None else None
        check(_lib.lib().pdgn_deconv_assemble_backward(F_, Fo, k, T, Fc, ptr(gC), ptr(gV), ptr(gB), ptr(dWi), ptr(dW2),
                                                       ptr(dWf), stream_of(ref)), "pdgn_deconv_assemble_backward")
        return dWi, dW2, dWf, None, None, None, None, None


class _ConvBN(nn.Module):

    def __init__(self, cin, cout, ksize):
        super().__init__()
        self.conv = nn.Conv2d(cin, cout, ksize, 1)
        self.bn = nn.BatchNorm2d(cout)


class _XyzTaps(torch.autograd.Function):

    @staticmethod
    def forward(ctx, Wx):
        a = Wx[:, 3:]
        return torch.cat([a, Wx[:, :3] - a], 0)

    @staticmethod
    def backward(ctx, g):
        n = g.shape[0] // 2
        g1, g2 = g[:n], g[n:]
        return torch.cat([g2, g1 - g2], 1)


class PointDeconv(nn.Module):

    def __init__(self, Fin, Fout, k, bilateral=True, softmax=True):
        super().__init__()
        if k % 2:
            raise ValueError("k must be even (the reference's view(B,N,C,2,k//2) :576 needs it)")
        self.k, self.Fin, self.Fout = k, Fin, Fout
        self.bilateral, self.softmax = bilateral, softmax
        self.conv2 = _ConvBN(2 * Fin, 2 * Fout, [1, 2 * k])
        if bilateral:
            self.conv_xyz = nn.Sequential(nn.Conv2d(6, 16, 1), nn.BatchNorm2d(16), nn.LeakyReLU(inplace=True))
            self.conv_fea = nn.Sequential(nn.Conv2d(2 * Fin, 16, 1), nn.BatchNorm2d(16),
                                          nn.LeakyReLU(inplace=True))
            self.conv_all = nn.Sequential(nn.Conv2d(16, 64, 1), nn.BatchNorm2d(64), nn.LeakyReLU(inplace=True),
                                          nn.Conv2d(64, 2 * Fin, 1), nn.BatchNorm2d(2 * Fin),
                                          nn.LeakyReLU(inplace=True))
        self.inte_conv_hk = nn.Sequential(nn.Conv2d(2 * Fin, 4 * Fin, [1, k // 2 + 1], [1, 1]),
                                          nn.BatchNorm2d(4 * Fin), nn.LeakyReLU(inplace=True))

    def _assemble(self):
        Fi, Fo, k = self.Fin, self.Fout, self.k
        T = k // 2 + 1
        Wi = self.inte_conv_hk[0].weight.squeeze(2)
        W2 = self.conv2.conv.weight.squeeze(2)
        W2a, W2b = W2[:, :, :k], W2[:, :, k:]
        blocks = [Wi[:, Fi:, :].permute(2, 0, 1).reshape(T * 4 * Fi, Fi),
                  (Wi[:, :Fi, :] - Wi[:, Fi:, :]).sum(2),
                  W2a[:, Fi:, :].permute(2, 0, 1).reshape(k * 2 * Fo, Fi),
                  (W2a[:, :Fi, :] - W2a[:, Fi:, :]).sum(2)]
        if self.bilateral:
            Wf = _w2d(self.conv_fea[0])
            blocks += [Wf[:, Fi:], Wf[:, :Fi] - Wf[:, Fi:]]
        Wcat = torch.cat(blocks, 0)
        P = k - T + 1
        Wb = W2b.reshape(2 * Fo, 2 * Fi, 2, P).permute(0, 3, 1, 2).reshape(2 * Fo, P * 4 * Fi)
        return Wcat, Wb, T, P

    def _weights_key(self, Fc):
        ws = [self.inte_conv_hk[0].weight, self.conv2.conv.weight] + ([self.conv_fea[0].weight, self.conv_all[3].weight] if self.bilateral else [])
        return (Fc, getattr(self, "_rows_hint", None)) + tuple((w.data_ptr(), w._version) for w in ws)

    def _assemble_now(self, Fc):
        Fi, Fo, k = self.Fin, self.Fout, self.k
        T = k // 2 + 1
        WcatC, WcatV, Wb = AssembleWeights.apply(self.inte_conv_hk[0].weight, self.conv2.conv.weight,
                                                 self.conv_fea[0].weight if self.bilateral else None, Fi, Fo, k, T, Fc)
        want_t = torch.is_grad_enabled() and WcatV.requires_grad
        with torch.no_grad():
            rows = getattr(self, "_rows_hint", None)
            pv = split_planes(WcatV.detach(), want_t, rows, dy_maxima_free=True)
            pb = split_planes(Wb.detach(), want_t, rows, x_maxima_free=self.bilateral and self.softmax)
            pa3 = (split_planes(_w2d(self.conv_all[3]).detach(), False, rows * self.k if rows else None, x_maxima_free=True)
                   if self.bilateral and _lib.gemm_mode() == "x2" else None)
            if pa3 is not None and pa3.parts_p != 2:
                pa3 = None
        return WcatC, WcatV, Wb, pv, pb, pa3

    def preassemble(self, Fc):
        self._pre = (self._weights_key(Fc), torch.is_grad_enabled(), self._assemble_now(Fc))

    def drop_preassembled(self):
        self._pre = None

    _FORWARD_HINTS = ("_rows_hint", "_pre")

    def forward_hints(self):
        return {k: self.__dict__[k] for k in self._FORWARD_HINTS if k in self.__dict__}

    def restore_forward_hints(self, hints):
        for k in self._FORWARD_HINTS:
            if k in hints:
                self.__dict__[k] = hints[k]
            else:
                self.__dict__.pop(k, None)

    def assembled(self, Fc):
        pre = getattr(self, "_pre", None)
        if pre is not None and pre[0] == self._weights_key(Fc) and (pre[1] or not torch.is_grad_enabled()):
            return pre[2]
        return self._assemble_now(Fc)

    def forward(self, x, pc=None, idx=None):
        out = self.forward_cl(x.transpose(1, 2).contiguous(),
                              pc.transpose(1, 2).contiguous() if pc is not None else None, idx=idx, x_cf=x)
        flush_bn_counters()
        return out.transpose(1, 2)

    def forward_cl(self, xt, pct=None, idx=None, x_cf=None, const=None, idx_ready=None):
        B, N, Fv = xt.shape
        Fi, Fo, k = self.Fin, self.Fout, self.k
        Fc = Fi - Fv
        training = self.training
        self._rows_hint = B * N
        knn_side = idx_ready
        if idx is None:
            idx, knn_side = start_feature_knn(xt, const, k, x_cf=x_cf)
        elif idx.dtype != I32:
            idx = idx.to(I32)
        idx = idx.contiguous()
        planes_v = planes_b = planes_a3 = None
        if xt.is_cuda:
            T = k // 2 + 1
            P = k - T + 1
            WcatC, WcatV, Wb, planes_v, planes_b, planes_a3 = self.assembled(Fc if const is not None else 0)
        else:
            Wcat, Wb, T, P = self._assemble()
            WcatC, WcatV = (Wcat[:, :Fc], Wcat[:, Fc:].contiguous()) if const is not None else (None, Wcat)
        o_i, o_ci = 0, T * 4 * Fi
        o_a = o_ci + 4 * Fi
        o_ca = o_a + k * 2 * Fo
        o_p = o_ca + 2 * Fo
        Yc = skinny_linear(const, WcatC) if const is not None else None
        fuse_stats = training and xt.is_cuda and Fi % 4 == 0 and Fv % 4 == 0
        specs_full = [(T, P, 4 * Fi, o_i, o_ci), (k, 1, 2 * Fo, o_a, o_ca)]
        biases = [self.inte_conv_hk[0].bias, self.conv2.conv.bias]
        if self.bilateral:
            specs_full.append((1, k, 16, o_p, o_p + 16))
            biases.append(self.conv_fea[0].bias)
        if Yc is not None and Yc.is_cuda:
            bb = SampleBias.apply(Yc, tuple((sp[0], sp[2], sp[3], sp[4]) for sp in specs_full), *biases)
            biases = list(torch.split(bb, [sp[2] for sp in specs_full], dim=1))
        elif Yc is not None:
            biases = [bias.unsqueeze(0) + Yc[:, sp[4]:sp[4] + sp[2]] + Yc[:, sp[3]:sp[3] + sp[0] * sp[2]].reshape(B, sp[0], sp[2]).sum(1)
                      for sp, bias in zip(specs_full, biases)]
        x2d = xt.reshape(B * N, Fv)
        specs = [(T, P, 4 * Fi, o_i, o_ci, fuse_stats)] + specs_full[1:]
        Y = linear_cl(x2d, WcatV, planes=planes_v).view(B, N, -1)
        if knn_side is not None:
            torch.cuda.current_stream(idx.device).wait_event(knn_side)
            idx.record_stream(torch.cuda.current_stream(idx.device))
        outs = EdgeGatherSum.apply(Y, idx, tuple(specs), *biases)
        inte_pre, a_pre = outs[0], outs[1]
        part_i = outs[-1] if fuse_stats else None
        w = None
        inte_max = inte_cmax = None
        if self.bilateral:
            Wx = _w2d(self.conv_xyz[0])
            Yx = linear_cl(pct.reshape(B * N, 3), _XyzTaps.apply(Wx)).view(B, N, -1)
            (xyz_pre,) = EdgeGatherSum.apply(Yx, idx, ((1, k, 16, 0, 16),), self.conv_xyz[0].bias)
            xyzf = bn_act(xyz_pre.view(-1, 16), self.conv_xyz[1], training)
            h = bn_act(outs[2].view(-1, 16), self.conv_fea[1], training, mul=xyzf)
            h, ph = linear_cl(h, _w2d(self.conv_all[0]), None, None, training)
            h = bn_act(h, self.conv_all[1], training, pre_bias=self.conv_all[0].bias, partials=ph)
            h, ph = linear_cl(h, _w2d(self.conv_all[3]), None, None, training, planes=planes_a3)
            if self.softmax:
                if planes_b is not None and planes_b.parts_p == 2:
                    inte, inte_max, inte_cmax = bilateral_weighting(h, self.conv_all[4], inte_pre.view(-1, 4 * Fi), self.inte_conv_hk[1], training, k,
                                                                    pre_bias_x=self.conv_all[3].bias, partials_u=part_i, partials_x=ph, want_max=True)
                else:
                    inte = bilateral_weighting(h, self.conv_all[4], inte_pre.view(-1, 4 * Fi), self.inte_conv_hk[1], training, k,
                                               pre_bias_x=self.conv_all[3].bias, partials_u=part_i, partials_x=ph)
            else:
                h = bn_act(h, self.conv_all[4], training, pre_bias=self.conv_all[3].bias, partials=ph)
                w = h.view(B, N, 2, P, 2 * Fi).permute(0, 1, 3, 4, 2).reshape(B * N * P, 4 * Fi)
                inte = bn_act(inte_pre.view(-1, 4 * Fi), self.inte_conv_hk[1], training, mul=w, partials=part_i)
        else:
            inte = bn_act(inte_pre.view(-1, 4 * Fi), self.inte_conv_hk[1], training, partials=part_i)
        out_pre = linear_cl(inte.view(B * N, P * 4 * Fi), Wb, None, a_pre.view(B * N, 2 * Fo), planes=planes_b, x_max=inte_max, x_cmax=inte_cmax)
        out = bn_act(out_pre, self.conv2.bn, training, act="relu", interleave_n=N)
        return out.view(B, 2 * N, Fo)


def upsample_edgeConv(Fin, Fout, k, num=None):
    return PointDeconv(Fin, Fout, k, bilateral=False)


def bilateral_upsample_edgeConv(Fin, Fout, k, num=None, softmax=True):
    return PointDeconv(Fin, Fout, k, bilateral=True, softmax=softmax)
```

pdgn_amd/fused.py:

```python
import os
import weakref
from typing import NamedTuple

import torch
from ._fn import Function

from . import _lib
from ._lib import check, ptr, require, stream_of

F32 = torch.float32
ACT = {"none": 0, "relu": 1, "leaky_relu": 2}


def _scratch_floats(L, rows, C):
    n = L.pdgn_bn_scratch_floats(rows, C)
    if n < 0:
        raise _lib.PdgnHipError("pdgn_bn_scratch_floats: argument outside the supported range")
    return n


class HandOver:
    def __init__(self, accepts):
        self.accepts, self.pending = accepts, {}

    def leave(self, tensor, payload=True):
        self.pending[tensor.data_ptr()] = (weakref.ref(tensor), payload)

    def take(self, tensor):
        ref, payload = self.pending.pop(tensor.data_ptr(), (None, None))
        src = ref() if ref is not None else None
        return payload if src is not None and (src is tensor or self.accepts(tensor, src)) else None

    def clear(self):
        self.pending.clear()

    def __len__(self):
        return len(self.pending)


_ZERO_COLSUM = HandOver(lambda dy, src: dy._base is src and dy.numel() == src.numel() and dy.shape[-1] == src.shape[-1])
mark_zero_colsum = _ZERO_COLSUM.leave


def has_zero_colsum(dy):
    return _ZERO_COLSUM.take(dy) is not None


def clear_zero_colsum():
    _ZERO_COLSUM.clear()
    _INPUT_GRADS.clear()
    _GRAD_MAXIMA.clear()


_GRAD_MAXIMA = HandOver(lambda dy, src: dy.numel() == src.numel() and dy.is_contiguous() and src.is_contiguous()
                        and (dy._base is src or (dy._base is not None and dy._base is src._base)))
mark_maxima, take_maxima = _GRAD_MAXIMA.leave, _GRAD_MAXIMA.take


_INPUT_GRADS = HandOver(lambda dy, src: (dy._base is src or dy._base is src._base) and dy.shape == src.shape)
_CLOSED_TAIL = os.environ.get("PDGN_CLOSED_TAIL", "1") == "1"
_STATS_MAX = os.environ.get("PDGN_STATS_MAX", "1") == "1"
_CLOSED_DW = os.environ.get("PDGN_CLOSED_DW", "1") == "1"


class DenseInput:

    def __init__(self, h, w):
        self.h, self.w = h, w


_NAN_SLOTS = {}


def _placeholder_with_input_grad(rows, C, dh, dw, device):
    pool = _NAN_SLOTS.get(device)
    if pool is None:
        pool = _NAN_SLOTS[device] = [torch.full((256,), float("nan"), dtype=F32, device=device), 0]
    i = pool[1]
    pool[1] = (i + 1) % 256
    tok = pool[0][i:i + 1].expand(rows, C)
    _INPUT_GRADS.leave(tok, (dh, dw))
    return tok


def is_placeholder(dy):
    return dy.dim() == 2 and dy.stride(0) == 0 and dy.stride(1) == 0 and dy.numel() > 1


def take_input_grad(dy):
    return _INPUT_GRADS.take(dy) if dy.stride(0) == 0 else None


_ARENA = {"buf": None, "off": 0, "need": 0, "owner": None}


def reset_zero_arena(device, owner):
    a = _ARENA
    if a["owner"] is not None:
        a["owner"].zero_arena_floats = max(getattr(a["owner"], "zero_arena_floats", 0), a["need"])
    size = getattr(owner, "zero_arena_floats", 0)
    a["buf"] = torch.zeros(size, dtype=F32, device=device) if size else None
    a["off"] = a["need"] = 0
    a["owner"] = owner


def release_zero_arena():
    a = _ARENA
    if a["owner"] is not None:
        a["owner"].zero_arena_floats = max(getattr(a["owner"], "zero_arena_floats", 0), a["need"])
    a["buf"] = None
    a["owner"] = None
    a["off"] = a["need"] = 0


def _zeros(shape, device):
    n = 1
    for d in shape:
        n *= d
    step = (n + 63) // 64 * 64
    a = _ARENA
    a["need"] += step
    buf = a["buf"]
    if buf is None or buf.device != device or a["off"] + step > buf.numel():
        return torch.zeros(shape, dtype=F32, device=device)
    v = buf[a["off"]:a["off"] + n].view(shape)
    a["off"] += step
    return v


_GROUP_COLSUM = os.environ.get("PDGN_GROUP_COLSUM", "1") == "1"


def group_colsum(x2d, group_rows=None):
    rows, C = x2d.shape
    gr = rows if group_rows is None else int(group_rows)
    if not (_GROUP_COLSUM and x2d.is_cuda and x2d.dtype == F32 and x2d.stride(1) == 1 and x2d.stride(0) % 4 == 0
            and x2d.data_ptr() % 16 == 0 and 16 <= C <= 1024 and (C & (C - 1)) == 0 and gr > 0 and rows % gr == 0
            and rows // gr <= 65535):
        return x2d.sum(dim=0, keepdim=True) if gr == rows else x2d.reshape(rows // gr, gr, C).sum(dim=1)
    out = _zeros((rows // gr, C), x2d.device)
    check(_lib.lib().pdgn_group_colsum(rows // gr, gr, C, ptr(x2d), x2d.stride(0), ptr(out), stream_of(x2d)), "pdgn_group_colsum")
    return out


def _bn_stats(L, x, rows, C, g, b, pre_bias, running_mean, running_var, training, momentum, eps, partials=None):
    stats = torch.empty(4 * C, dtype=F32, device=x.device)
    pb = pre_bias.detach().contiguous() if pre_bias is not None else None
    block = None
    if isinstance(partials, tuple):
        partials, block = partials
    if training and block is not None:
        nparts = partials.shape[0]
        nd = L.pdgn_bn_blocks_scratch_doubles(C, nparts)
        scr = torch.empty(nd, dtype=torch.float64, device=x.device) if nd > 0 else None
        check(L.pdgn_bn_stats_from_gemm_partials(rows, C, nparts, block, eps, momentum, ptr(g), ptr(b), ptr(pb),
                                                 ptr(running_mean), ptr(running_var), ptr(partials), ptr(stats), ptr(scr), stream_of(x)),
              "pdgn_bn_stats_from_gemm_partials")
    elif training and partials is not None:
        check(L.pdgn_bn_stats_from_partials(rows, C, eps, momentum, ptr(g), ptr(b), ptr(pb), ptr(running_mean), ptr(running_var), ptr(partials),
                                            ptr(stats), stream_of(x)), "pdgn_bn_stats_from_partials")
    elif training:
        scratch = torch.empty(_scratch_floats(L, rows, C), dtype=F32, device=x.device)
        check(L.pdgn_bn_stats(rows, C, eps, momentum, ptr(x), ptr(g), ptr(b), ptr(pb), ptr(running_mean), ptr(running_var), ptr(scratch), ptr(stats),
                              stream_of(x)), "pdgn_bn_stats")
    else:
        check(L.pdgn_bn_eval_stats(C, eps, ptr(g), ptr(b), ptr(pb), ptr(running_mean),
                                   ptr(running_var), ptr(stats), stream_of(x)), "pdgn_bn_eval_stats")
    return stats


_NO_FOLD = os.environ.get("PDGN_FOLD_BIAS", "1") == "0"


def _fold_pre_bias(x2d, pre_bias, training):
    if pre_bias is not None and (_NO_FOLD or (not training and torch.is_grad_enabled() and pre_bias.requires_grad)):
        return x2d + pre_bias, None
    return x2d, pre_bias


def _pre_bias_grad(ctx_has, C, device):
    return _zeros((C,), device) if ctx_has else None


class BNActCL(Function):

    @staticmethod
    def forward(ctx, x, gamma, beta, running_mean, running_var, training, momentum, eps, act, mul, pre_bias=None,
                partials=None, interleave_n=0):
        rows, C = x.shape
        x = x.contiguous()
        L = _lib.lib()
        g, b = gamma.detach().contiguous(), beta.detach().contiguous()
        stats = _bn_stats(L, x, rows, C, g, b, pre_bias, running_mean, running_var, training, momentum, eps, partials)
        ctx.has_pre_bias = pre_bias is not None
        mul_c = mul.contiguous() if mul is not None else None
        y = torch.empty((rows * 2, C // 2), dtype=F32, device=x.device) if interleave_n else torch.empty_like(x)
        check(L.pdgn_bn_act_forward(rows, C, act, ptr(x), ptr(stats), ptr(mul_c), ptr(y), int(interleave_n), stream_of(x)), "pdgn_bn_act_forward")
        ctx.save_for_backward(x, stats, mul_c)
        ctx.cfg = (rows, C, act, bool(training), mul is not None and mul.requires_grad, int(interleave_n))
        return y

    @staticmethod
    def backward(ctx, dy):
        x, stats, mul = ctx.saved_tensors
        rows, C, act, training, need_dmul, inter = ctx.cfg
        dy = dy.contiguous()
        L = _lib.lib()
        scratch = torch.empty(_scratch_floats(L, rows, C), dtype=F32, device=x.device)
        bs = torch.empty(2 * C, dtype=F32, device=x.device)
        dx = torch.empty_like(x)
        dmul = torch.empty_like(x) if need_dmul else None
        check(L.pdgn_bn_act_backward(rows, C, act, int(training), ptr(x), ptr(dy), ptr(mul),
                                     ptr(stats), ptr(scratch), ptr(bs), ptr(dx), ptr(dmul), inter, stream_of(x)), "pdgn_bn_act_backward")
        if training:
            mark_zero_colsum(dx)
        return (dx, bs[C:], bs[:C], None, None, None, None, None, None, dmul, _pre_bias_grad(ctx.has_pre_bias, C, x.device),
                None, None)


_PENDING_COUNTS = {}
_HOLD_COUNTS = [False]


def hold_bn_counters(on):
    old, _HOLD_COUNTS[0] = _HOLD_COUNTS[0], bool(on)
    return old


def flush_bn_counters():
    if _HOLD_COUNTS[0]:
        return
    if _PENDING_COUNTS:
        tensors = list(_PENDING_COUNTS.keys())
        torch._foreach_add_(tensors, [int(v) for v in _PENDING_COUNTS.values()])
        _PENDING_COUNTS.clear()


def bn_act(x2d, bn, training, act="leaky_relu", mul=None, pre_bias=None, partials=None, interleave_n=0):
    if training and bn.track_running_stats:
        _PENDING_COUNTS[bn.num_batches_tracked] = _PENDING_COUNTS.get(bn.num_batches_tracked, 0) + 1
    x2d, pre_bias = _fold_pre_bias(x2d, pre_bias, training)
    if x2d.shape[1] % 4:
        if pre_bias is not None:
            x2d = x2d + pre_bias
        y = torch.nn.functional.batch_norm(x2d, bn.running_mean, bn.running_var, bn.weight, bn.bias, training,
                                           bn.momentum, bn.eps)
        y = {"none": lambda t: t, "relu": torch.relu, "leaky_relu": torch.nn.functional.leaky_relu}[act](y)
        y = y * mul if mul is not None else y
        return interleave_rows(y, interleave_n) if interleave_n else y
    if interleave_n and (mul is not None or not x2d.is_cuda):
        return interleave_rows(bn_act(x2d, bn, training, act, mul, pre_bias, partials), interleave_n)
    return BNActCL.apply(x2d, bn.weight, bn.bias, bn.running_mean, bn.running_var, training, bn.momentum, bn.eps,
                         ACT[act], mul, pre_bias, partials, interleave_n)


def interleave_rows(y2d, n):
    rows, c2 = y2d.shape
    return y2d.view(rows // n, n, c2 // 2, 2).permute(0, 3, 1, 2).reshape(rows * 2, c2 // 2)


_OWN_MIN_ROWS = 1024
_TN_BIG = os.environ.get("PDGN_TN_BIG", "1") == "1"


def _tn_big_max():
    return (1 << 22) if _lib.matrix_core_mode() else (1 << 20)


def _pad_cols(t, mult=4):
    c = t.shape[1]
    if c % mult == 0 and t.stride(1) == 1 and t.stride(0) % 4 == 0 and t.data_ptr() % 16 == 0:
        return t
    if c % mult == 0:
        return t.contiguous()
    return torch.nn.functional.pad(t, (0, mult - c % mult)).contiguous()


GEMM_LOG = None


_PLANES = os.environ.get("PDGN_PLANES", "1") == "1"


class Planes:
    __slots__ = ("p", "t", "shape", "parts_p", "parts_t")

    def __init__(self, p, t, shape, parts_p=3, parts_t=3):
        self.p, self.t, self.shape, self.parts_p, self.parts_t = p, t, shape, parts_p, parts_t


def two_part(m, n, k, scan_bytes):
    return _lib.gemm_mode() == "x2" and bool(_lib.lib().pdgn_gemm_two_part(m, n, k, scan_bytes))


def two_part_planes(m, n, k, scan_bytes):
    return _lib.gemm_mode() == "x2" and bool(_lib.lib().pdgn_gemm_two_part_planes(m, n, k, scan_bytes))


def _slots(t):
    if _lib.gemm_mode() == "x2":
        _lib.ensure_scale_slots(t.device)


def split_planes(w, want_t, rows=None, dy_maxima_free=False, x_maxima_free=False):
    _slots(w)
    mode = _lib.gemm_mode()
    if (not (_PLANES and w.is_cuda and w.dim() == 2 and mode != "fp32") or w.shape[0] % 4 or w.shape[1] % 4 or w.stride(1) != 1
            or w.stride(0) % 4 or w.data_ptr() % 16):
        return None
    n, k = w.shape
    ldp, ldt = (k + 7) // 8 * 8, (n + 7) // 8 * 8
    parts_p = 2 if rows and two_part_planes(rows, n, k, 0 if x_maxima_free else rows * k * 4) else 3
    parts_t = 2 if rows and want_t and two_part_planes(rows, k, n, 0 if dy_maxima_free else rows * n * 4) else 3

    def planes(parts, rows_, ld):
        buf = torch.empty(parts * rows_ * ld + 2 * rows_ + 8, dtype=torch.int16, device=w.device)
        return buf[:parts * rows_ * ld].view(parts, rows_, ld)
    P = planes(parts_p, n, ldp)
    PT = planes(parts_t, k, ldt) if want_t else None
    L = _lib.lib()
    st = stream_of(w)
    if parts_p == parts_t or not want_t:
        fn = L.pdgn_split_bf16x3 if parts_p == 3 else L.pdgn_split_f16x2
        check(fn(n, k, ptr(w), w.stride(0), ptr(P), ldp, n * ldp, ptr(PT), ldt, k * ldt if want_t else 0, st), "pdgn_split")
    else:
        for parts, args in ((parts_p, (ptr(P), ldp, n * ldp, None, 0, 0)),
                            (parts_t, (None, 0, 0, ptr(PT), ldt, k * ldt))):
            fn = L.pdgn_split_bf16x3 if parts == 3 else L.pdgn_split_f16x2
            check(fn(n, k, ptr(w), w.stride(0), *args, st), "pdgn_split")
    return Planes(P, PT, (n, k), parts_p, parts_t)


def _maxima_ok(t):
    return (_lib.gemm_mode() == "x2" and t.is_cuda and t.dim() == 2 and t.stride(1) == 1 and t.dtype == F32 and t.shape[1] % 4 == 0
            and t.stride(0) % 4 == 0 and t.data_ptr() % 16 == 0)


def operand_maxima(t, rows=True, cols=False):
    if not _maxima_ok(t) or not (rows or cols):
        return (None, None) if (rows and cols) else None
    rm = torch.empty((t.shape[0],), dtype=torch.int32, device=t.device) if rows else None
    cm = torch.empty((t.shape[1],), dtype=torch.int32, device=t.device) if cols else None
    check(_lib.lib().pdgn_absmax_rows_cols(t.shape[0], t.shape[1], ptr(t), t.stride(0), ptr(rm), ptr(cm), stream_of(t)), "pdgn_absmax_rows_cols")
    return (rm, cm) if (rows and cols) else (rm if rows else cm)


def row_maxima_buffer(rows, device):
    return torch.empty((rows,), dtype=torch.int32, device=device)


def _hand_maxima(L, ma, mw=None):
    if ma is not None or mw is not None:
        L.pdgn_gemm_set_operand_scales(ptr(ma), ptr(mw))


def _tail_workspace(L, m, n, k, with_stats, device, parts=None):
    if parts is not None:
        need = L.pdgn_gemm_nt_ps_workspace_floats(m, n, k, parts, 1 if with_stats else 0)
    else:
        need = L.pdgn_gemm_tail_workspace_floats(m, n, k, 1 if with_stats else 0)
    if need <= 0:
        return None
    ws = torch.empty(need, dtype=F32, device=device)
    check(L.pdgn_gemm_set_tail_workspace(ptr(ws), need), "pdgn_gemm_set_tail_workspace")
    return ws


def _rp_takes(m, n, k, parts, plain):
    return parts == 2 and plain and _lib.lib().pdgn_gemm_nt_ps_row_panel(m, n, k, 2, 1) == 1


def planes_fit(P, m, n, k, with_stats=False, plain=False, panel=None):
    return (P.shape[0] == 3 or not with_stats or (_rp_takes(m, n, k, P.shape[0], plain) if panel is None else panel)
            or (_lib.lib().pdgn_gemm_nt_config(m, n, k, 1) & 15) == 0)


def _nt_frame(entry, a, n, k, bias, addend, want_stats, max_a, parts, stat_rows, launch):
    _slots(a)
    if GEMM_LOG is not None:
        GEMM_LOG.append(entry)
    m = a.shape[0]
    ap = _pad_cols(a)
    L = _lib.lib()
    out = torch.empty((m, n), dtype=F32, device=a.device)
    part = torch.empty((stat_rows(L), 3 * n), dtype=F32, device=a.device) if want_stats else None
    b = bias.detach().contiguous() if bias is not None else None
    if addend is not None:
        addend = _pad_cols(addend)
    ws = _tail_workspace(L, m, n, k, want_stats, a.device, parts=parts)
    _hand_maxima(L, max_a)
    launch(L, ap, b, addend, addend.stride(0) if addend is not None else 0, out, part)
    return out, part


def gemm_nt_planes(a, P, n, k, bias=None, addend=None, want_stats=False, max_a=None):
    m, parts, plain = a.shape[0], P.shape[0], 1 if (bias is None and addend is None) else 0

    def launch(L, ap, b, add, ldadd, out, part):
        check(L.pdgn_gemm_nt_ps(m, n, k, ptr(ap), ap.stride(0), ptr(P), P.shape[2], P.shape[1] * P.shape[2], parts, ptr(b), ptr(add), ldadd,
                                ptr(out), n, ptr(part), None, 0, 1, 0, None, 0, stream_of(a)), "pdgn_gemm_nt_ps")
    out, part = _nt_frame(("nt", m, n, k), a, n, k, bias, addend, want_stats, max_a, parts,
                          lambda L: L.pdgn_gemm_nt_ps_stat_rows(m, n, k, parts, plain), launch)
    return (out, part) if want_stats else out


def gemm_nt(a, w, bias=None, addend=None, want_stats=False, w_transposed=False, max_a=None):
    m, k = a.shape
    n = w.shape[1] if w_transposed else w.shape[0]
    kp, np_ = (k + 3) // 4 * 4, (n + 3) // 4 * 4
    wp = _pad_cols(w)
    rows = (kp - k) if w_transposed else (np_ - n)
    if rows:
        wp = torch.nn.functional.pad(wp, (0, 0, 0, rows))
    if np_ != n:
        bias = torch.nn.functional.pad(bias, (0, np_ - n)) if bias is not None else None
        addend = torch.nn.functional.pad(addend, (0, np_ - n)) if addend is not None else None
    name = "pdgn_gemm_nn" if w_transposed else "pdgn_gemm_nt"

    def launch(L, ap, b, add, ldadd, out, part):
        check(getattr(L, name)(m, np_, kp, ptr(ap), ap.stride(0), ptr(wp), wp.stride(0), ptr(b), ptr(add), ldadd, ptr(out), np_, ptr(part),
                               stream_of(a)), name)
    out, part = _nt_frame(("nn" if w_transposed else "nt", m, n, k), a, np_, kp, bias, addend, want_stats, max_a, None,
                          lambda L: L.pdgn_gemm_nt_stat_rows(m, np_, kp), launch)
    if np_ != n:
        out = out[:, :n].contiguous()
    return (out, part) if want_stats else out


def gemm_tn(dy, x, max_dy=None, max_x=None):
    _slots(dy)
    m, n = dy.shape
    k = x.shape[1]
    if GEMM_LOG is not None:
        GEMM_LOG.append(("tn", m, n, k))
    dyp, xp = _pad_cols(dy), _pad_cols(x)
    np_, kp = dyp.shape[1], xp.shape[1]
    L = _lib.lib()
    if _TN_BIG and np_ >= 64 and kp >= 64 and (65536 if (m < 150000 or not _lib.matrix_core_mode()) else 16384) <= np_ * kp <= _tn_big_max():
        need = L.pdgn_gemm_tn_big_workspace_floats(m, np_, kp)
        if need > 0:
            ws = torch.empty(need, dtype=F32, device=dy.device)
            check(L.pdgn_gemm_set_tail_workspace(ptr(ws), need), "pdgn_gemm_set_tail_workspace")
            dwp = torch.empty((np_, kp), dtype=F32, device=dy.device)
        else:
            dwp = _zeros((np_, kp), dy.device)
        _hand_maxima(L, max_dy, max_x)
        check(L.pdgn_gemm_tn_big(m, np_, kp, ptr(dyp), dyp.stride(0), ptr(xp), xp.stride(0), ptr(dwp), 0 if need > 0 else 1, stream_of(dy)),
              "pdgn_gemm_tn_big")
    else:
        dyp, xp = (t if t.stride(0) == t.shape[1] else t.contiguous() for t in (dyp, xp))
        dwp = _zeros((np_, kp), dy.device)
        check(L.pdgn_gemm_tn(m, np_, kp, ptr(dyp), ptr(xp), ptr(dwp), stream_of(dy)), "pdgn_gemm_tn")
    return dwp if (np_ == n and kp == k) else dwp[:n, :k]


def _thin_ok(x, n, k):
    return (k <= 4 and n % 4 == 0 and n <= 1024) or (n <= 4 and k % 4 == 0 and k <= 1024)


def thin_nt(x, w, wrs, wcs, n, bias=None, want_stats=False):
    m, k = x.shape
    if GEMM_LOG is not None:
        GEMM_LOG.append(("thin", m, n, k))
    x = x if (x.stride(1) == 1 and (k <= 4 or (x.stride(0) % 4 == 0 and x.data_ptr() % 16 == 0))) else x.contiguous()
    L = _lib.lib()
    out = torch.empty((m, n), dtype=F32, device=x.device)
    part = None
    if want_stats and k <= 4:
        part = torch.empty((L.pdgn_thin_stat_rows(m), 3 * n), dtype=F32, device=x.device)
    b = bias.detach().contiguous() if bias is not None else None
    check(L.pdgn_thin_nt(m, n, k, ptr(x), x.stride(0), ptr(w), wrs, wcs, ptr(b), ptr(out), n, ptr(part), stream_of(x)), "pdgn_thin_nt")
    return (out, part) if want_stats else out


def thin_tn(dy, x, want_db):
    m, n = dy.shape
    k = x.shape[1]
    if GEMM_LOG is not None:
        GEMM_LOG.append(("thin_tn", m, n, k))
    dw = _zeros((n, k), dy.device)
    db = _zeros((n,), dy.device) if want_db else None
    L = _lib.lib()
    if k <= 4:
        check(L.pdgn_thin_tn(m, k, n, ptr(x), x.stride(0), ptr(dy), dy.stride(0), ptr(dw), 1, k, ptr(None), ptr(db), stream_of(dy)), "pdgn_thin_tn")
    else:
        check(L.pdgn_thin_tn(m, n, k, ptr(dy), dy.stride(0), ptr(x), x.stride(0), ptr(dw), k, 1, ptr(db), ptr(None), stream_of(dy)), "pdgn_thin_tn")
    return dw, db


_PLANES_MIN_ROWS = 4096


class DenseRoute(NamedTuple):
    route: str
    stats: bool = False
    block_rows: int = 0
    x_maxima: bool = False


def dense_route(x, weight, bias=None, addend=None, planes=None, want_stats=False):
    m, (n, k) = x.shape[0], weight.shape
    if not x.is_cuda:
        return DenseRoute("torch")
    plain = bias is None and addend is None
    if planes is not None and m >= _PLANES_MIN_ROWS and planes.shape == (n, k) and x.shape[1] == k and k % 4 == 0:
        parts = planes.p.shape[0]
        panel = _rp_takes(m, n, k, parts, plain)
        if planes_fit(planes.p, m, n, k, want_stats, plain, panel):
            block = _lib.lib().pdgn_gemm_nt_ps_stat_block_rows(m, n, k, parts, 1 if plain else 0) if want_stats else 0
            return DenseRoute("planes", bool(want_stats), block, parts == 2 and not panel)
    if m < _OWN_MIN_ROWS:
        return DenseRoute("torch")
    if addend is None and weight.is_contiguous() and _thin_ok(x, n, k):
        stats = bool(want_stats) and k <= 4
        return DenseRoute("thin", stats, _lib.lib().pdgn_thin_stat_block_rows() if stats else 0)
    stats = bool(want_stats) and n % 4 == 0
    return DenseRoute("own", stats, _lib.lib().pdgn_gemm_nt_stat_block_rows(m, (n + 3) // 4 * 4, (k + 3) // 4 * 4) if stats else 0)


class LinearCL(Function):
# ... 647 lines not shown
```

Before: 3.119 million points/s.

## Fuse xyz and feature branch gathers and paired BN-act into joint kernels

The bilateral branch used to run two separate edge-gather-sum passes (feature and xyz), two BN stats finalizes and two bn_act passes before multiplying the results. These are now combined: one paired gather kernel emits both pre-activations with stats partials, one kernel finalizes both BNs, and one forward kernel computes act(bn(a))*act(bn(b)), with a matching paired backward. The aim is to cut kernel launches and intermediate memory traffic. It adds a new code path, gated by an env flag that defaults on, plus a fallback to the old route.

```diff
diff --git a/include/pdgn_hip.h b/include/pdgn_hip.h
--- a/include/pdgn_hip.h
+++ b/include/pdgn_hip.h
@@ -12,7 +12,7 @@
 
 typedef void *pdgn_stream_t;
 
-#define PDGN_ABI_VERSION 41
+#define PDGN_ABI_VERSION 42
 int pdgn_abi_version(void);
 
 int pdgn_knnquery(int b, int n, int m, int nsample, const float *xyz, const float *new_xyz,
@@ -96,6 +96,21 @@
 int pdgn_bn_act_backward(long long rows, int c, int act, int training, const float *x,
                          const float *dy, const float *mul, const float *stats, float *scratch,
                          float *bsums, float *dx, float *dmul, int interleave_n, pdgn_stream_t stream);
+
+int pdgn_pair_gather_stats(int b, int n, int k, int T, int P, int C, const float *Ya, int ldya, int offa, int offca,
+                           const float *Yb, int ldyb, int offb, int offcb, const int32_t *idx, const float *bias_a,
+                           int bias_a_bstride, const float *bias_b, int bias_b_bstride, float *out_a, float *out_b,
+                           float *part_a, float *part_b, pdgn_stream_t stream);
+int pdgn_bn_pair_stats(long long rows, int c, float eps_a, float momentum_a, const float *gamma_a, const float *beta_a,
+                       const float *pre_bias_a, float *running_mean_a, float *running_var_a, const float *part_a,
+                       const float *pivot_a, float *stats_a, float eps_b, float momentum_b, const float *gamma_b,
+                       const float *beta_b, const float *pre_bias_b, float *running_mean_b, float *running_var_b,
+                       const float *part_b, const float *pivot_b, float *stats_b, pdgn_stream_t stream);
+int pdgn_bn_act_pair_forward(long long rows, int c, int act, const float *xa, const float *stats_a, const float *xb,
+                             const float *stats_b, float *h, pdgn_stream_t stream);
+int pdgn_bn_act_pair_backward(long long rows, int c, int act, int training, const float *xa, const float *xb, const float *dh,
+                              const float *stats_a, const float *stats_b, float *scratch_a, float *scratch_b, float *bsums_a,
+                              float *bsums_b, float *dxa, float *dxb, pdgn_stream_t stream);
 
 long long pdgn_bn_maxpool_scratch_floats(int b, int c);
 int pdgn_bn_act_maxpool(int b, int n, int c, int act, const float *x, const float *stats, float *scratch,
diff --git a/pdgn_amd/csrc/bn_elem.h b/pdgn_amd/csrc/bn_elem.h
--- /dev/null
+++ b/pdgn_amd/csrc/bn_elem.h
@@ -0,0 +1,116 @@
+#pragma once
+#include "common.h"
+
+#define ACT_NONE 0
+#define ACT_RELU 1
+#define ACT_LEAKY 2
+
+__device__ __forceinline__ float act_fwd(float z, int act) {
+    if (act == ACT_RELU) return fmaxf(z, 0.f);
+    if (act == ACT_LEAKY) return z > 0.f ? z : 0.01f * z;
+    return z;
+}
+__device__ __forceinline__ float act_grad(float z, int act) {
+    if (act == ACT_RELU) return z > 0.f ? 1.f : 0.f;
+    if (act == ACT_LEAKY) return z > 0.f ? 1.f : 0.01f;
+    return 1.f;
+}
+
+__device__ __forceinline__ void bn_stat_accum(float x, float pv, float &s, float &q) {
+    const float d = x - pv;
+    s += d;
+    q = __fmaf_rn(d, d, q);
+}
+__device__ __forceinline__ float bn_z(float x, float sc, float sh) { return __fmaf_rn(x, sc, sh); }
+__device__ __forceinline__ void bn_bwd_accum(float dz, float x, float mu, float is, float &s, float &q) {
+    s += dz;
+    q = __fmaf_rn(dz, (x - mu) * is, q);
+}
+__device__ __forceinline__ float bn_bwd_dx(float sc, float dz, float ca, float cb, float x) {
+    return __fmaf_rn(sc, dz, -ca) - cb * x;
+}
+
+#define FIN_CH 4
+#define FIN_PL 64
+
+__device__ __forceinline__ void fin_reduce2(const float *__restrict__ part, int nparts, size_t ld, int c, int C, bool ok,
+                                            double (*red)[FIN_CH], double (*red2)[FIN_CH], double &s1, double &s2) {
+    const int cl = threadIdx.x % FIN_CH, pl = threadIdx.x / FIN_CH;
+    double a = 0, b = 0;
+    if (ok) {
+        int p = pl;
+        for (; p + 3 * FIN_PL < nparts; p += 4 * FIN_PL) {
+            const float *q = part + (size_t)p * ld + c;
+            const float a0 = q[0], a1 = q[(size_t)FIN_PL * ld], a2 = q[(size_t)2 * FIN_PL * ld], a3 = q[(size_t)3 * FIN_PL * ld];
+            const float b0 = q[C], b1 = q[(size_t)FIN_PL * ld + C], b2 = q[(size_t)2 * FIN_PL * ld + C], b3 = q[(size_t)3 * FIN_PL * ld + C];
+            a += ((double)a0 + (double)a1) + ((double)a2 + (double)a3);
+            b += ((double)b0 + (double)b1) + ((double)b2 + (double)b3);
+        }
+        for (; p < nparts; p += FIN_PL) {
+            a += (double)part[(size_t)p * ld + c];
+            b += (double)part[(size_t)p * ld + C + c];
+        }
+    }
+    red[pl][cl] = a;
+    red2[pl][cl] = b;
+    __syncthreads();
+    for (int h = FIN_PL / 2; h > 0; h >>= 1) {
+        if (pl < h) {
+            red[pl][cl] += red[pl + h][cl];
+            red2[pl][cl] += red2[pl + h][cl];
+        }
+        __syncthreads();
+    }
+    s1 = red[0][cl];
+    s2 = red2[0][cl];
+}
+
+__device__ __forceinline__ void cl_finalize_body(
+    long long R, int C, int nparts, float eps, float momentum, const float *__restrict__ part,
+    const float *__restrict__ gamma, const float *__restrict__ beta, const float *__restrict__ pre_bias,
+    float *__restrict__ running_mean, float *__restrict__ running_var, float *__restrict__ stats,
+    const float *__restrict__ pivot, double (*red)[FIN_CH], double (*red2)[FIN_CH]) {
+    const int c = blockIdx.x * FIN_CH + threadIdx.x % FIN_CH;
+    const bool ok = c < C;
+    double s1, s2;
+    fin_reduce2(part, nparts, (size_t)2 * C, c, C, ok, red, red2, s1, s2);
+    if (!ok || threadIdx.x >= FIN_CH) return;
+    const double ms = s1 / (double)R;
+    double var = s2 / (double)R - ms * ms;
+    var = var < 0 ? 0 : var;
+    const double mean = ms + (pivot ? (double)pivot[c] : 0.0);
+    const float invstd = (float)(1.0 / sqrt(var + (double)eps));
+    const float g = gamma ? gamma[c] : 1.f, b = beta ? beta[c] : 0.f;
+    const float scale = g * invstd;
+    stats[c] = scale;
+    stats[C + c] = b - (float)mean * scale;
+    stats[2 * C + c] = (float)mean;
+    stats[3 * C + c] = invstd;
+    if (running_mean) {
+        const double unbiased = R > 1 ? var * (double)R / (double)(R - 1) : var;
+        const float mb = (float)mean + (pre_bias ? pre_bias[c] : 0.f);
+        running_mean[c] = (1.f - momentum) * running_mean[c] + momentum * mb;
+        running_var[c] = (1.f - momentum) * running_var[c] + momentum * (float)unbiased;
+    }
+}
+
+__device__ __forceinline__ void cl_bwd_finalize_body(long long R, int C, int nparts, int training,
+                                                     const float *__restrict__ part, const float *__restrict__ stats,
+                                                     float *__restrict__ bsums, float *__restrict__ coef,
+                                                     double (*red)[FIN_CH], double (*red2)[FIN_CH]) {
+    const int c = blockIdx.x * FIN_CH + threadIdx.x % FIN_CH;
+    const bool ok = c < C;
+    double s1, s2;
+    fin_reduce2(part, nparts, (size_t)2 * C, c, C, ok, red, red2, s1, s2);
+    if (!ok || threadIdx.x >= FIN_CH) return;
+    bsums[c] = (float)s1;
+    bsums[C + c] = (float)s2;
+    float ca = 0.f, cb = 0.f;
+    if (training) {
+        const float sc = stats[c], mu = stats[2 * C + c], is = stats[3 * C + c];
+        cb = sc * is * (float)(s2 / (double)R);
+        ca = sc * (float)(s1 / (double)R) - cb * mu;
+    }
+    coef[c] = ca;
+    coef[C + c] = cb;
+}
diff --git a/pdgn_amd/csrc/bnact.hip b/pdgn_amd/csrc/bnact.hip
--- a/pdgn_amd/csrc/bnact.hip
+++ b/pdgn_amd/csrc/bnact.hip
@@ -1,20 +1,7 @@
 #include "common.h"
 
 #include "bn_geom.h"
-#define ACT_NONE 0
-#define ACT_RELU 1
-#define ACT_LEAKY 2
-
-__device__ __forceinline__ float act_fwd(float z, int act) {
-    if (act == ACT_RELU) return fmaxf(z, 0.f);
-    if (act == ACT_LEAKY) return z > 0.f ? z : 0.01f * z;
-    return z;
-}
-__device__ __forceinline__ float act_grad(float z, int act) {
-    if (act == ACT_RELU) return z > 0.f ? 1.f : 0.f;
-    if (act == ACT_LEAKY) return z > 0.f ? 1.f : 0.01f;
-    return 1.f;
-}
+#include "bn_elem.h"
 
 struct ClGeom {
     int cg, cgb, rl;
@@ -40,18 +27,14 @@
             for (int u = 0; u < 4; ++u) v[u] = *reinterpret_cast<const float4 *>(X + (r + (long long)u * rl) * C);
 #pragma unroll
             for (int u = 0; u < 4; ++u) {
-                const float dx = v[u].x - pv.x, dy = v[u].y - pv.y, dz = v[u].z - pv.z, dw = v[u].w - pv.w;
-                s.x += dx; s.y += dy; s.z += dz; s.w += dw;
-                q.x = __fmaf_rn(dx, dx, q.x); q.y = __fmaf_rn(dy, dy, q.y);
-                q.z = __fmaf_rn(dz, dz, q.z); q.w = __fmaf_rn(dw, dw, q.w);
+                bn_stat_accum(v[u].x, pv.x, s.x, q.x); bn_stat_accum(v[u].y, pv.y, s.y, q.y);
+                bn_stat_accum(v[u].z, pv.z, s.z, q.z); bn_stat_accum(v[u].w, pv.w, s.w, q.w);
             }
         }
         for (; r < r1; r += rl) {
             const float4 v = *reinterpret_cast<const float4 *>(X + r * C);
-            const float dx = v.x - pv.x, dy = v.y - pv.y, dz = v.z - pv.z, dw = v.w - pv.w;
-            s.x += dx; s.y += dy; s.z += dz; s.w += dw;
-            q.x = __fmaf_rn(dx, dx, q.x); q.y = __fmaf_rn(dy, dy, q.y);
-            q.z = __fmaf_rn(dz, dz, q.z); q.w = __fmaf_rn(dw, dw, q.w);
+            bn_stat_accum(v.x, pv.x, s.x, q.x); bn_stat_accum(v.y, pv.y, s.y, q.y);
+            bn_stat_accum(v.z, pv.z, s.z, q.z); bn_stat_accum(v.w, pv.w, s.w, q.w);
         }
     }
     red[0][threadIdx.x] = s;
@@ -69,8 +52,6 @@
     }
 }
 
-#define FIN_CH 4
-#define FIN_PL 64
 
 __device__ __forceinline__ double fin_reduce(const float *__restrict__ part, int nparts, size_t ld, int c, bool ok,
                                              double (*red)[FIN_CH]) {
@@ -94,66 +75,13 @@
     return red[0][cl];
 }
 
-__device__ __forceinline__ void fin_reduce2(const float *__restrict__ part, int nparts, size_t ld, int c, int C, bool ok,
-                                            double (*red)[FIN_CH], double (*red2)[FIN_CH], double &s1, double &s2) {
-    const int cl = threadIdx.x % FIN_CH, pl = threadIdx.x / FIN_CH;
-    double a = 0, b = 0;
-    if (ok) {
-        int p = pl;
-        for (; p + 3 * FIN_PL < nparts; p += 4 * FIN_PL) {
-            const float *q = part + (size_t)p * ld + c;
-            const float a0 = q[0], a1 = q[(size_t)FIN_PL * ld], a2 = q[(size_t)2 * FIN_PL * ld], a3 = q[(size_t)3 * FIN_PL * ld];
-            const float b0 = q[C], b1 = q[(size_t)FIN_PL * ld + C], b2 = q[(size_t)2 * FIN_PL * ld + C], b3 = q[(size_t)3 * FIN_PL * ld + C];
-            a += ((double)a0 + (double)a1) + ((double)a2 + (double)a3);
-            b += ((double)b0 + (double)b1) + ((double)b2 + (double)b3);
-        }
-        for (; p < nparts; p += FIN_PL) {
-            a += (double)part[(size_t)p * ld + c];
-            b += (double)part[(size_t)p * ld + C + c];
-        }
-    }
-    red[pl][cl] = a;
-    red2[pl][cl] = b;
-    __syncthreads();
-    for (int h = FIN_PL / 2; h > 0; h >>= 1) {
-        if (pl < h) {
-            red[pl][cl] += red[pl + h][cl];
-            red2[pl][cl] += red2[pl + h][cl];
-        }
-        __syncthreads();
-    }
-    s1 = red[0][cl];
-    s2 = red2[0][cl];
-}
-
 __global__ __launch_bounds__(FIN_CH * FIN_PL) void cl_finalize_kernel(
     long long R, int C, int nparts, float eps, float momentum, const float *__restrict__ part,
     const float *__restrict__ gamma, const float *__restrict__ beta, const float *__restrict__ pre_bias,
     float *__restrict__ running_mean, float *__restrict__ running_var, float *__restrict__ stats,
     const float *__restrict__ pivot) {
     __shared__ double red[FIN_PL][FIN_CH], red2[FIN_PL][FIN_CH];
-    const int c = blockIdx.x * FIN_CH + threadIdx.x % FIN_CH;
-    const bool ok = c < C;
-    double s1, s2;
-    fin_reduce2(part, nparts, (size_t)2 * C, c, C, ok, red, red2, s1, s2);
-    if (!ok || threadIdx.x >= FIN_CH) return;
-    const double ms = s1 / (double)R;
-    double var = s2 / (double)R - ms * ms;
-    var = var < 0 ? 0 : var;
-    const double mean = ms + (pivot ? (double)pivot[c] : 0.0);
-    const float invstd = (float)(1.0 / sqrt(var + (double)eps));
-    const float g = gamma ? gamma[c] : 1.f, b = beta ? beta[c] : 0.f;
-    const float scale = g * invstd;
-    stats[c] = scale;
-    stats[C + c] = b - (float)mean * scale;
-    stats[2 * C + c] = (float)mean;
-    stats[3 * C + c] = invstd;
-    if (running_mean) {
-        const double unbiased = R > 1 ? var * (double)R / (double)(R - 1) : var;
-        const float mb = (float)mean + (pre_bias ? pre_bias[c] : 0.f);
-        running_mean[c] = (1.f - momentum) * running_mean[c] + momentum * mb;
-        running_var[c] = (1.f - momentum) * running_var[c] + momentum * (float)unbiased;
-    }
+    cl_finalize_body(R, C, nparts, eps, momentum, part, gamma, beta, pre_bias, running_mean, running_var, stats, pivot, red, red2);
 }
 
 __global__ __launch_bounds__(FIN_CH * FIN_PL) void cl_finalize_blocks_kernel(
@@ -372,8 +300,8 @@
             const long long rr = r + (long long)u * rl;
             if (rr < r1) {
                 float4 o;
-                o.x = act_fwd(__fmaf_rn(v[u].x, sc.x, sh.x), act); o.y = act_fwd(__fmaf_rn(v[u].y, sc.y, sh.y), act);
-                o.z = act_fwd(__fmaf_rn(v[u].z, sc.z, sh.z), act); o.w = act_fwd(__fmaf_rn(v[u].w, sc.w, sh.w), act);
+                o.x = act_fwd(bn_z(v[u].x, sc.x, sh.x), act); o.y = act_fwd(bn_z(v[u].y, sc.y, sh.y), act);
+                o.z = act_fwd(bn_z(v[u].z, sc.z, sh.z), act); o.w = act_fwd(bn_z(v[u].w, sc.w, sh.w), act);
                 if (has_mul) { o.x *= m[u].x; o.y *= m[u].y; o.z *= m[u].z; o.w *= m[u].w; }
                 if (pn) {
                     long long ra, rb;
@@ -431,10 +359,10 @@
                 if (rb + (long long)u * rl < r1) {
                     if (has_mul) { g[u].x *= m[u].x; g[u].y *= m[u].y; g[u].z *= m[u].z; g[u].w *= m[u].w; }
                     float dz;
-                    dz = g[u].x * act_grad(__fmaf_rn(v[u].x, sc.x, sh.x), act); s.x += dz; q.x = __fmaf_rn(dz, (v[u].x - mu.x) * is.x, q.x);
-                    dz = g[u].y * act_grad(__fmaf_rn(v[u].y, sc.y, sh.y), act); s.y += dz; q.y = __fmaf_rn(dz, (v[u].y - mu.y) * is.y, q.y);
-                    dz = g[u].z * act_grad(__fmaf_rn(v[u].z, sc.z, sh.z), act); s.z += dz; q.z = __fmaf_rn(dz, (v[u].z - mu.z) * is.z, q.z);
-                    dz = g[u].w * act_grad(__fmaf_rn(v[u].w, sc.w, sh.w), act); s.w += dz; q.w = __fmaf_rn(dz, (v[u].w - mu.w) * is.w, q.w);
+                    dz = g[u].x * act_grad(bn_z(v[u].x, sc.x, sh.x), act); bn_bwd_accum(dz, v[u].x, mu.x, is.x, s.x, q.x);
+                    dz = g[u].y * act_grad(bn_z(v[u].y, sc.y, sh.y), act); bn_bwd_accum(dz, v[u].y, mu.y, is.y, s.y, q.y);
+                    dz = g[u].z * act_grad(bn_z(v[u].z, sc.z, sh.z), act); bn_bwd_accum(dz, v[u].z, mu.z, is.z, s.z, q.z);
+                    dz = g[u].w * act_grad(bn_z(v[u].w, sc.w, sh.w), act); bn_bwd_accum(dz, v[u].w, mu.w, is.w, s.w, q.w);
                 }
             }
         }
@@ -460,21 +388,7 @@
                                                                          float *__restrict__ bsums,
                                                                          float *__restrict__ coef) {
     __shared__ double red[FIN_PL][FIN_CH], red2[FIN_PL][FIN_CH];
-    const int c = blockIdx.x * FIN_CH + threadIdx.x % FIN_CH;
-    const bool ok = c < C;
-    double s1, s2;
-    fin_reduce2(part, nparts, (size_t)2 * C, c, C, ok, red, red2, s1, s2);
-    if (!ok || threadIdx.x >= FIN_CH) return;
-    bsums[c] = (float)s1;
-    bsums[C + c] = (float)s2;
-    float ca = 0.f, cb = 0.f;
-    if (training) {
-        const float sc = stats[c], mu = stats[2 * C + c], is = stats[3 * C + c];
-        cb = sc * is * (float)(s2 / (double)R);
-        ca = sc * (float)(s1 / (double)R) - cb * mu;
-    }
-    coef[c] = ca;
-    coef[C + c] = cb;
+    cl_bwd_finalize_body(R, C, nparts, training, part, stats, bsums, coef, red, red2);
 }
 
 __global__ __launch_bounds__(BN_THREADS) void cl_bwd_apply_kernel(long long R, int C, int cgb, int rows_per_block, int act,
@@ -521,10 +435,10 @@
                 float o[4], om[4];
 #pragma unroll
                 for (int j = 0; j < 4; ++j) {
-                    const float z = __fmaf_rn(v[u][j], sc[j], sh[j]);
+                    const float z = bn_z(v[u][j], sc[j], sh[j]);
                     om[j] = g[u][j] * act_fwd(z, act);
                     const float dz = (has_mul ? g[u][j] * m[u][j] : g[u][j]) * act_grad(z, act);
-                    o[j] = __fmaf_rn(sc[j], dz, -ca[j]) - cb[j] * v[u][j];
+                    o[j] = bn_bwd_dx(sc[j], dz, ca[j], cb[j], v[u][j]);
                 }
                 *reinterpret_cast<float4 *>(dx + rr * C + cgi * 4) = *reinterpret_cast<float4 *>(o);
                 if (want_dmul) *reinterpret_cast<float4 *>(dmul + rr * C + cgi * 4) = *reinterpret_cast<float4 *>(om);
diff --git a/pdgn_amd/csrc/pair.hip b/pdgn_amd/csrc/pair.hip
--- /dev/null
+++ b/pdgn_amd/csrc/pair.hip
@@ -0,0 +1,342 @@
+#include "bn_elem.h"
+#include "bn_geom.h"
+
+struct PairSrc {
+    const float *Y, *bias;
+    float *out, *part;
+    int ldy, off, offc, bstride;
+};
+
+__device__ __forceinline__ float4 pair_add4(float4 a, float4 b) { return make_float4(a.x + b.x, a.y + b.y, a.z + b.z, a.w + b.w); }
+
+__device__ __forceinline__ float4 pair_row(const PairSrc &S, int c, unsigned bs, unsigned bn, unsigned src_row) {
+    float4 acc = S.bias ? *reinterpret_cast<const float4 *>(S.bias + (size_t)bs * S.bstride + c) : make_float4(0.f, 0.f, 0.f, 0.f);
+    if (S.offc >= 0) acc = pair_add4(acc, *reinterpret_cast<const float4 *>(S.Y + (size_t)bn * S.ldy + S.offc + c));
+    return pair_add4(acc, *reinterpret_cast<const float4 *>(S.Y + (size_t)src_row * S.ldy + S.off + c));
+}
+
+__device__ __forceinline__ void pair_stat4(float4 v, float4 pv, float4 &s, float4 &q) {
+    bn_stat_accum(v.x, pv.x, s.x, q.x); bn_stat_accum(v.y, pv.y, s.y, q.y);
+    bn_stat_accum(v.z, pv.z, s.z, q.z); bn_stat_accum(v.w, pv.w, s.w, q.w);
+}
+
+__global__ __launch_bounds__(BN_THREADS) void pair_gather_stats_kernel(unsigned R, unsigned n, int k, unsigned P, int C, int cgb,
+                                                                       int rows_per_block, PairSrc A, PairSrc B,
+                                                                       const int32_t *__restrict__ idx) {
+    __shared__ float4 red[4][BN_THREADS];
+    const int cgl = threadIdx.x % cgb, rlane = threadIdx.x / cgb, rl = BN_THREADS / cgb;
+    const int cgi = blockIdx.x * cgb + cgl;
+    const bool cok = cgi * 4 < C;
+    const int c = cgi * 4;
+    const unsigned r0 = blockIdx.y * (unsigned)rows_per_block;
+    const unsigned r1 = min(R, r0 + (unsigned)rows_per_block);
+    const float4 zero = make_float4(0.f, 0.f, 0.f, 0.f);
+    float4 sa = zero, qa = zero, sb = zero, qb = zero;
+    if (cok) {
+        const unsigned i0 = (unsigned)idx[0];
+        const float4 pva = pair_row(A, c, 0, 0, i0), pvb = pair_row(B, c, 0, 0, i0);
+        unsigned r = r0 + rlane;
+        for (; r + 3u * rl < r1; r += 4u * rl) {
+            unsigned bn[4], bs[4], src[4];
+#pragma unroll
+            for (int u = 0; u < 4; ++u) {
+                const unsigned rr = r + (unsigned)u * rl;
+                bn[u] = rr / P;
+                bs[u] = bn[u] / n;
+                src[u] = bs[u] * n + (unsigned)idx[(size_t)bn[u] * k + (rr - bn[u] * P)];
+            }
+            float4 va[4], vb[4];
+#pragma unroll
+            for (int u = 0; u < 4; ++u) {
+                va[u] = pair_row(A, c, bs[u], bn[u], src[u]);
+                vb[u] = pair_row(B, c, bs[u], bn[u], src[u]);
+            }
+#pragma unroll
+            for (int u = 0; u < 4; ++u) {
+                const size_t o = (size_t)(r + (unsigned)u * rl) * C + c;
+                *reinterpret_cast<float4 *>(A.out + o) = va[u];
+                *reinterpret_cast<float4 *>(B.out + o) = vb[u];
+                pair_stat4(va[u], pva, sa, qa);
+                pair_stat4(vb[u], pvb, sb, qb);
+            }
+        }
+        for (; r < r1; r += rl) {
+            const unsigned bn = r / P, bs = bn / n;
+            const unsigned src = bs * n + (unsigned)idx[(size_t)bn * k + (r - bn * P)];
+            const float4 va = pair_row(A, c, bs, bn, src), vb = pair_row(B, c, bs, bn, src);
+            *reinterpret_cast<float4 *>(A.out + (size_t)r * C + c) = va;
+            *reinterpret_cast<float4 *>(B.out + (size_t)r * C + c) = vb;
+            pair_stat4(va, pva, sa, qa);
+            pair_stat4(vb, pvb, sb, qb);
+        }
+    }
+    red[0][threadIdx.x] = sa;
+    red[1][threadIdx.x] = qa;
+    red[2][threadIdx.x] = sb;
+    red[3][threadIdx.x] = qb;
+    __syncthreads();
+    if (rlane == 0 && cok) {
+        for (int j = 1; j < rl; ++j) {
+            sa = pair_add4(sa, red[0][j * cgb + cgl]);
+            qa = pair_add4(qa, red[1][j * cgb + cgl]);
+            sb = pair_add4(sb, red[2][j * cgb + cgl]);
+            qb = pair_add4(qb, red[3][j * cgb + cgl]);
+        }
+        float *Pa = A.part + (size_t)blockIdx.y * 2 * C, *Pb = B.part + (size_t)blockIdx.y * 2 * C;
+        *reinterpret_cast<float4 *>(Pa + c) = sa;
+        *reinterpret_cast<float4 *>(Pa + C + c) = qa;
+        *reinterpret_cast<float4 *>(Pb + c) = sb;
+        *reinterpret_cast<float4 *>(Pb + C + c) = qb;
+    }
+}
+
+struct PairFin {
+    const float *part, *gamma, *beta, *pre_bias, *pivot;
+    float *running_mean, *running_var, *stats;
+    float eps, momentum;
+};
+
+__global__ __launch_bounds__(FIN_CH * FIN_PL) void pair_finalize_kernel(long long R, int C, int nparts, PairFin A, PairFin B) {
+    __shared__ double red[FIN_PL][FIN_CH], red2[FIN_PL][FIN_CH];
+    const PairFin &F = blockIdx.y ? B : A;
+    cl_finalize_body(R, C, nparts, F.eps, F.momentum, F.part, F.gamma, F.beta, F.pre_bias, F.running_mean, F.running_var, F.stats,
+                     F.pivot, red, red2);
+}
+
+__global__ __launch_bounds__(BN_THREADS) void pair_apply_kernel(long long R, int C, int cgb, int rows_per_block, int act,
+                                                                const float *__restrict__ xa, const float *__restrict__ stats_a,
+                                                                const float *__restrict__ xb, const float *__restrict__ stats_b,
+                                                                float *__restrict__ h) {
+    const int cgl = threadIdx.x % cgb, rlane = threadIdx.x / cgb, rl = BN_THREADS / cgb;
+    const int cgi = blockIdx.x * cgb + cgl;
+    if (cgi * 4 >= C) return;
+    const long long r0 = (long long)blockIdx.y * rows_per_block;
+    const long long r1 = min(R, r0 + rows_per_block);
+    const float4 sca = *reinterpret_cast<const float4 *>(stats_a + cgi * 4), sha = *reinterpret_cast<const float4 *>(stats_a + C + cgi * 4);
+    const float4 scb = *reinterpret_cast<const float4 *>(stats_b + cgi * 4), shb = *reinterpret_cast<const float4 *>(stats_b + C + cgi * 4);
+    for (long long r = r0 + rlane; r < r1; r += 4 * rl) {
+        float4 va[4], vb[4];
+#pragma unroll
+        for (int u = 0; u < 4; ++u) {
+            const long long rr = r + (long long)u * rl;
+            if (rr < r1) {
+                va[u] = *reinterpret_cast<const float4 *>(xa + rr * C + cgi * 4);
+                vb[u] = *reinterpret_cast<const float4 *>(xb + rr * C + cgi * 4);
+            }
+        }
+#pragma unroll
+        for (int u = 0; u < 4; ++u) {
+            const long long rr = r + (long long)u * rl;
+            if (rr < r1) {
+                float4 o;
+                o.x = act_fwd(bn_z(va[u].x, sca.x, sha.x), act) * act_fwd(bn_z(vb[u].x, scb.x, shb.x), act);
+                o.y = act_fwd(bn_z(va[u].y, sca.y, sha.y), act) * act_fwd(bn_z(vb[u].y, scb.y, shb.y), act);
+                o.z = act_fwd(bn_z(va[u].z, sca.z, sha.z), act) * act_fwd(bn_z(vb[u].z, scb.z, shb.z), act);
+                o.w = act_fwd(bn_z(va[u].w, sca.w, sha.w), act) * act_fwd(bn_z(vb[u].w, scb.w, shb.w), act);
+                *reinterpret_cast<float4 *>(h + rr * C + cgi * 4) = o;
+            }
+        }
+    }
+}
+
+__device__ __forceinline__ void pair_dz(float dh, float za, float zb, int act, float &dza, float &dzb) {
+    dza = (dh * act_fwd(zb, act)) * act_grad(za, act);
+    dzb = (dh * act_fwd(za, act)) * act_grad(zb, act);
+}
+
+struct PairBwd {
+    const float *x, *stats;
+    float *part;
+    const float *coef;
+    float *dx;
+};
+
+__global__ __launch_bounds__(BN_THREADS) void pair_bwd_reduce_kernel(long long R, int C, int cgb, int rows_per_block, int act,
+                                                                     const float *__restrict__ dh, PairBwd A, PairBwd B) {
+    __shared__ float4 red[4][BN_THREADS];
+    const int cgl = threadIdx.x % cgb, rlane = threadIdx.x / cgb, rl = BN_THREADS / cgb;
+    const int cgi = blockIdx.x * cgb + cgl;
+    const bool cok = cgi * 4 < C;
+    const long long r0 = (long long)blockIdx.y * rows_per_block;
+    const long long r1 = min(R, r0 + rows_per_block);
+    float sa[4] = {0.f, 0.f, 0.f, 0.f}, qa[4] = {0.f, 0.f, 0.f, 0.f}, sb[4] = {0.f, 0.f, 0.f, 0.f}, qb[4] = {0.f, 0.f, 0.f, 0.f};
+    if (cok) {
+        float sca[4], sha[4], mua[4], isa[4], scb[4], shb[4], mub[4], isb[4];
+        *reinterpret_cast<float4 *>(sca) = *reinterpret_cast<const float4 *>(A.stats + cgi * 4);
+        *reinterpret_cast<float4 *>(sha) = *reinterpret_cast<const float4 *>(A.stats + C + cgi * 4);
+        *reinterpret_cast<float4 *>(mua) = *reinterpret_cast<const float4 *>(A.stats + 2 * C + cgi * 4);
+        *reinterpret_cast<float4 *>(isa) = *reinterpret_cast<const float4 *>(A.stats + 3 * C + cgi * 4);
+        *reinterpret_cast<float4 *>(scb) = *reinterpret_cast<const float4 *>(B.stats + cgi * 4);
+        *reinterpret_cast<float4 *>(shb) = *reinterpret_cast<const float4 *>(B.stats + C + cgi * 4);
+        *reinterpret_cast<float4 *>(mub) = *reinterpret_cast<const float4 *>(B.stats + 2 * C + cgi * 4);
+        *reinterpret_cast<float4 *>(isb) = *reinterpret_cast<const float4 *>(B.stats + 3 * C + cgi * 4);
+        for (long long rb = r0 + rlane; rb < r1; rb += 4LL * rl) {
+            float va[4][4], vb[4][4], g[4][4];
+#pragma unroll
+            for (int u = 0; u < 4; ++u) {
+                const long long r = rb + (long long)u * rl;
+                if (r < r1) {
+                    *reinterpret_cast<float4 *>(va[u]) = *reinterpret_cast<const float4 *>(A.x + r * C + cgi * 4);
+                    *reinterpret_cast<float4 *>(vb[u]) = *reinterpret_cast<const float4 *>(B.x + r * C + cgi * 4);
+                    *reinterpret_cast<float4 *>(g[u]) = *reinterpret_cast<const float4 *>(dh + r * C + cgi * 4);
+                }
+            }
+#pragma unroll
+            for (int u = 0; u < 4; ++u) {
+                if (rb + (long long)u * rl < r1) {
+#pragma unroll
+                    for (int j = 0; j < 4; ++j) {
+                        float dza, dzb;
+                        pair_dz(g[u][j], bn_z(va[u][j], sca[j], sha[j]), bn_z(vb[u][j], scb[j], shb[j]), act, dza, dzb);
+                        bn_bwd_accum(dza, va[u][j], mua[j], isa[j], sa[j], qa[j]);
+                        bn_bwd_accum(dzb, vb[u][j], mub[j], isb[j], sb[j], qb[j]);
+                    }
+                }
+            }
+        }
+    }
+    red[0][threadIdx.x] = *reinterpret_cast<float4 *>(sa);
+    red[1][threadIdx.x] = *reinterpret_cast<float4 *>(qa);
+    red[2][threadIdx.x] = *reinterpret_cast<float4 *>(sb);
+    red[3][threadIdx.x] = *reinterpret_cast<float4 *>(qb);
+    __syncthreads();
+    if (rlane == 0 && cok) {
+        float4 s4a = *reinterpret_cast<float4 *>(sa), q4a = *reinterpret_cast<float4 *>(qa);
+        float4 s4b = *reinterpret_cast<float4 *>(sb), q4b = *reinterpret_cast<float4 *>(qb);
+        for (int j = 1; j < rl; ++j) {
+            s4a = pair_add4(s4a, red[0][j * cgb + cgl]);
+            q4a = pair_add4(q4a, red[1][j * cgb + cgl]);
+            s4b = pair_add4(s4b, red[2][j * cgb + cgl]);
+            q4b = pair_add4(q4b, red[3][j * cgb + cgl]);
+        }
+        float *Pa = A.part + (size_t)blockIdx.y * 2 * C, *Pb = B.part + (size_t)blockIdx.y * 2 * C;
+        *reinterpret_cast<float4 *>(Pa + cgi * 4) = s4a;
+        *reinterpret_cast<float4 *>(Pa + C + cgi * 4) = q4a;
+        *reinterpret_cast<float4 *>(Pb + cgi * 4) = s4b;
+        *reinterpret_cast<float4 *>(Pb + C + cgi * 4) = q4b;
+    }
+}
+
+struct PairBwdFin {
+    const float *part, *stats;
+    float *bsums, *coef;
+};
+
+__global__ __launch_bounds__(FIN_CH * FIN_PL) void pair_bwd_finalize_kernel(long long R, int C, int nparts, int training,
+                                                                           PairBwdFin A, PairBwdFin B) {
+    __shared__ double red[FIN_PL][FIN_CH], red2[FIN_PL][FIN_CH];
+    const PairBwdFin &F = blockIdx.y ? B : A;
+    cl_bwd_finalize_body(R, C, nparts, training, F.part, F.stats, F.bsums, F.coef, red, red2);
+}
+
+__global__ __launch_bounds__(BN_THREADS) void pair_bwd_apply_kernel(long long R, int C, int cgb, int rows_per_block, int act,
+                                                                    const float *__restrict__ dh, PairBwd A, PairBwd B) {
+    const int cgl = threadIdx.x % cgb, rlane = threadIdx.x / cgb, rl = BN_THREADS / cgb;
+    const int cgi = blockIdx.x * cgb + cgl;
+    if (cgi * 4 >= C) return;
+    const long long r0 = (long long)blockIdx.y * rows_per_block;
+    const long long r1 = min(R, r0 + rows_per_block);
+    float sca[4], sha[4], caa[4], cba[4], scb[4], shb[4], cab[4], cbb[4];
+    *reinterpret_cast<float4 *>(sca) = *reinterpret_cast<const float4 *>(A.stats + cgi * 4);
+    *reinterpret_cast<float4 *>(sha) = *reinterpret_cast<const float4 *>(A.stats + C + cgi * 4);
+    *reinterpret_cast<float4 *>(caa) = *reinterpret_cast<const float4 *>(A.coef + cgi * 4);
+    *reinterpret_cast<float4 *>(cba) = *reinterpret_cast<const float4 *>(A.coef + C + cgi * 4);
+    *reinterpret_cast<float4 *>(scb) = *reinterpret_cast<const float4 *>(B.stats + cgi * 4);
+    *reinterpret_cast<float4 *>(shb) = *reinterpret_cast<const float4 *>(B.stats + C + cgi * 4);
+    *reinterpret_cast<float4 *>(cab) = *reinterpret_cast<const float4 *>(B.coef + cgi * 4);
+    *reinterpret_cast<float4 *>(cbb) = *reinterpret_cast<const float4 *>(B.coef + C + cgi * 4);
+    for (long long r = r0 + rlane; r < r1; r += 4 * rl) {
+        float va[4][4], vb[4][4], g[4][4];
+#pragma unroll
+        for (int u = 0; u < 4; ++u) {
+            const long long rr = r + (long long)u * rl;
+            if (rr < r1) {
+                *reinterpret_cast<float4 *>(va[u]) = *reinterpret_cast<const float4 *>(A.x + rr * C + cgi * 4);
+                *reinterpret_cast<float4 *>(vb[u]) = *reinterpret_cast<const float4 *>(B.x + rr * C + cgi * 4);
+                *reinterpret_cast<float4 *>(g[u]) = *reinterpret_cast<const float4 *>(dh + rr * C + cgi * 4);
+            }
+        }
+#pragma unroll
+        for (int u = 0; u < 4; ++u) {
+            const long long rr = r + (long long)u * rl;
+            if (rr < r1) {
+                float oa[4], ob[4];
+#pragma unroll
+                for (int j = 0; j < 4; ++j) {
+                    float dza, dzb;
+                    pair_dz(g[u][j], bn_z(va[u][j], sca[j], sha[j]), bn_z(vb[u][j], scb[j], shb[j]), act, dza, dzb);
+                    oa[j] = bn_bwd_dx(sca[j], dza, caa[j], cba[j], va[u][j]);
+                    ob[j] = bn_bwd_dx(scb[j], dzb, cab[j], cbb[j], vb[u][j]);
+                }
+                *reinterpret_cast<float4 *>(A.dx + rr * C + cgi * 4) = *reinterpret_cast<float4 *>(oa);
+                *reinterpret_cast<float4 *>(B.dx + rr * C + cgi * 4) = *reinterpret_cast<float4 *>(ob);
+            }
+        }
+    }
+}
+
+static bool pair_src_ok(const float *Y, int ldy, int off, int offc, int C, const float *bias, int bstride) {
+    return Y && ldy >= 4 && ldy % 4 == 0 && off >= 0 && off % 4 == 0 && off + C <= ldy && (offc < 0 || (offc % 4 == 0 && offc + C <= ldy)) &&
+           ((size_t)Y & 15) == 0 && (!bias || (bstride >= 0 && bstride % 4 == 0 && ((size_t)bias & 15) == 0));
+}
+
+extern "C" int pdgn_pair_gather_stats(int b, int n, int k, int T, int P, int C, const float *Ya, int ldya, int offa, int offca,
+                                      const float *Yb, int ldyb, int offb, int offcb, const int32_t *idx, const float *bias_a,
+                                      int bias_a_bstride, const float *bias_b, int bias_b_bstride, float *out_a, float *out_b,
+                                      float *part_a, float *part_b, pdgn_stream_t stream) {
+    if (T != 1 || b < 1 || n < 1 || k < 1 || P < 1 || P > k || C < 4 || C % 4) return PDGN_ERR_INVALID;
+    if (!pair_src_ok(Ya, ldya, offa, offca, C, bias_a, bias_a_bstride) || !pair_src_ok(Yb, ldyb, offb, offcb, C, bias_b, bias_b_bstride))
+        return PDGN_ERR_INVALID;
+    if (!idx || !out_a || !out_b || !part_a || !part_b) return PDGN_ERR_INVALID;
+    if ((long long)b * n * k > 0x7fffffffLL) return PDGN_ERR_INVALID;
+    const long long R = (long long)b * n * P;
+    int cgb, gx, gy, rpb;
+    cl_geometry(R, C, &cgb, &gx, &gy, &rpb);
+    const PairSrc A = {Ya, bias_a, out_a, part_a, ldya, offa, offca, bias_a_bstride};
+    const PairSrc B = {Yb, bias_b, out_b, part_b, ldyb, offb, offcb, bias_b_bstride};
+    hipLaunchKernelGGL(pair_gather_stats_kernel, dim3(gx, gy), dim3(BN_THREADS), 0, (hipStream_t)stream, (unsigned)R, (unsigned)n, k,
+                       (unsigned)P, C, cgb, rpb, A, B, idx);
+    return pdgn_launch_status();
+}
+
+extern "C" int pdgn_bn_pair_stats(long long rows, int c, float eps_a, float momentum_a, const float *gamma_a, const float *beta_a,
+                                  const float *pre_bias_a, float *running_mean_a, float *running_var_a, const float *part_a,
+                                  const float *pivot_a, float *stats_a, float eps_b, float momentum_b, const float *gamma_b,
+                                  const float *beta_b, const float *pre_bias_b, float *running_mean_b, float *running_var_b,
+                                  const float *part_b, const float *pivot_b, float *stats_b, pdgn_stream_t stream) {
+    if (rows < 1 || c < 4 || c % 4 || !part_a || !part_b || !stats_a || !stats_b) return PDGN_ERR_INVALID;
+    int cgb, gx, gy, rpb;
+    cl_geometry(rows, c, &cgb, &gx, &gy, &rpb);
+    const PairFin A = {part_a, gamma_a, beta_a, pre_bias_a, pivot_a, running_mean_a, running_var_a, stats_a, eps_a, momentum_a};
+    const PairFin B = {part_b, gamma_b, beta_b, pre_bias_b, pivot_b, running_mean_b, running_var_b, stats_b, eps_b, momentum_b};
+    hipLaunchKernelGGL(pair_finalize_kernel, dim3(cdiv(c, FIN_CH), 2), dim3(FIN_CH * FIN_PL), 0, (hipStream_t)stream, rows, c, gy, A, B);
+    return pdgn_launch_status();
+}
+
+extern "C" int pdgn_bn_act_pair_forward(long long rows, int c, int act, const float *xa, const float *stats_a, const float *xb,
+                                        const float *stats_b, float *h, pdgn_stream_t stream) {
+    if (rows < 1 || c < 4 || c % 4 || act < 0 || act > 2 || !xa || !xb || !stats_a || !stats_b || !h) return PDGN_ERR_INVALID;
+    int cgb, gx, gy, rpb;
+    cl_geometry(rows, c, &cgb, &gx, &gy, &rpb);
+    hipLaunchKernelGGL(pair_apply_kernel, dim3(gx, gy), dim3(BN_THREADS), 0, (hipStream_t)stream, rows, c, cgb, rpb, act, xa, stats_a,
+                       xb, stats_b, h);
+    return pdgn_launch_status();
+}
+
+extern "C" int pdgn_bn_act_pair_backward(long long rows, int c, int act, int training, const float *xa, const float *xb,
+                                         const float *dh, const float *stats_a, const float *stats_b, float *scratch_a,
+                                         float *scratch_b, float *bsums_a, float *bsums_b, float *dxa, float *dxb,
+                                         pdgn_stream_t stream) {
+    if (rows < 1 || c < 4 || c % 4 || act < 0 || act > 2) return PDGN_ERR_INVALID;
+    if (!xa || !xb || !dh || !stats_a || !stats_b || !scratch_a || !scratch_b || !bsums_a || !bsums_b || !dxa || !dxb) return PDGN_ERR_INVALID;
+    hipStream_t s = (hipStream_t)stream;
+    int cgb, gx, gy, rpb;
+    cl_geometry(rows, c, &cgb, &gx, &gy, &rpb);
+    float *coef_a = scratch_a + (size_t)gy * 2 * c, *coef_b = scratch_b + (size_t)gy * 2 * c;
+    const PairBwd A = {xa, stats_a, scratch_a, coef_a, dxa}, B = {xb, stats_b, scratch_b, coef_b, dxb};
+    hipLaunchKernelGGL(pair_bwd_reduce_kernel, dim3(gx, gy), dim3(BN_THREADS), 0, s, rows, c, cgb, rpb, act, dh, A, B);
+    const PairBwdFin FA = {scratch_a, stats_a, bsums_a, coef_a}, FB = {scratch_b, stats_b, bsums_b, coef_b};
+    hipLaunchKernelGGL(pair_bwd_finalize_kernel, dim3(cdiv(c, FIN_CH), 2), dim3(FIN_CH * FIN_PL), 0, s, rows, c, gy, training, FA, FB);
+    hipLaunchKernelGGL(pair_bwd_apply_kernel, dim3(gx, gy), dim3(BN_THREADS), 0, s, rows, c, cgb, rpb, act, dh, A, B);
+    return pdgn_launch_status();
+}
diff --git a/pdgn_amd/deconv.py b/pdgn_amd/deconv.py
--- a/pdgn_amd/deconv.py
+++ b/pdgn_amd/deconv.py
@@ -8,7 +8,7 @@
 from . import _lib
 from . import streams as _streams
 from ._lib import check, ptr, require, stream_of
-from .fused import (Planes, split_planes, skinny_linear, _zeros, bilateral_weighting, bn_act,
+from .fused import (Planes, split_planes, skinny_linear, _zeros, bilateral_weighting, bn_act, bn_act_pair, branch_pair_route,
                     small_sequential, bn_act_maxpool, bn_softmax_slots_permute, flush_bn_counters,
                     has_zero_colsum, linear_cl, softmax_slots_permute, DenseInput, group_colsum, mark_maxima, row_maxima_buffer)
 from .fused import _STATS_MAX as STATS_MAX
@@ -73,6 +73,13 @@
     return idx, ready
 
 
+def _bias_arg(bias, C):
+    if bias is not None and bias.dim() == 2 and bias.stride(1) == 1:
+        return bias.detach(), bias.stride(0)
+    bias_c = bias.detach().contiguous() if bias is not None else None
+    return bias_c, (C if (bias is not None and bias.dim() == 2) else 0)
+
+
 class EdgeGatherSum(Function):
 
     @staticmethod
@@ -81,27 +88,7 @@
         require(idx, "idx", I32, 3)
         b, n, ldy = Y.shape
         k = idx.shape[2]
-        outs, partials = [], []
-        L = _lib.lib()
-        for spec, bias in zip(specs, biases):
-            T, P, C, off, offc = spec[:5]
-            out = torch.empty((b, n, P, C), dtype=F32, device=Y.device)
-            if bias is not None and bias.dim() == 2 and bias.stride(1) == 1:
-                bias_c, bstride = bias.detach(), bias.stride(0)
-            else:
-                bias_c = bias.detach().contiguous() if bias is not None else None
-                bstride = C if (bias is not None and bias.dim() == 2) else 0
-            if len(spec) > 5 and spec[5]:
-                scr = torch.empty(L.pdgn_bn_scratch_floats(b * n * P, C), dtype=F32, device=Y.device)
-                check(L.pdgn_window_gather_sum_stats(b, n, k, ldy, T, P, C, off, offc, ptr(Y), ptr(idx), ptr(bias_c),
-                                                     bstride, ptr(out), ptr(scr), stream_of(Y)),
-                      "pdgn_window_gather_sum_stats")
-                partials.append(scr)
-            else:
-                check(L.pdgn_window_gather_sum(b, n, k, ldy, T, P, C, off, offc, ptr(Y), ptr(idx),
-                                               ptr(bias_c), bstride, ptr(out), stream_of(Y)),
-                      "pdgn_window_gather_sum")
-            outs.append(out)
+        outs, partials = _gather_sum_forward(Y, idx, specs, biases)
         specs = tuple(tuple(spec[:5]) for spec in specs)
         ctx.mark_non_differentiable(*partials)
         ctx.set_materialize_grads(False)
@@ -113,41 +100,124 @@
     @staticmethod
     def backward(ctx, *douts):
         (idx,) = ctx.saved_tensors
-        b, n, ldy, k = ctx.shape
-        douts = [d if d is not None else torch.zeros((b, n, P, C), dtype=F32, device=idx.device)
-                 for d, (T, P, C, off, offc) in zip(douts, ctx.specs)]
-        L = _lib.lib()
-        covered = sum(T * C + (C if offc >= 0 else 0) for (T, P, C, off, offc) in ctx.specs)
-        vec_ok = ldy % 4 == 0 and k <= 31 and all(C % 4 == 0 and off % 4 == 0 and (offc < 0 or offc % 4 == 0)
-                                                 for (T, P, C, off, offc) in ctx.specs)
-        dbias = []
-        if vec_ok and covered == ldy:
-            rowptr, edges = transposed_graph(idx)
-            dY = torch.empty((b, n, ldy), dtype=F32, device=idx.device)
-            dmax = row_maxima_buffer(b * n, idx.device) if (_lib.gemm_mode() == "x2" and b * n * ldy >= (1 << 24)) else None
-            first = 1
-            for (T, P, C, off, offc), dout, hb in zip(ctx.specs, douts, ctx.has_bias):
-                hb = 3 if hb == 1 and has_zero_colsum(dout) else hb
-                dout = dout.contiguous()
-                check(L.pdgn_window_gather_sum_backward_csr(b, n, k, ldy, T, P, C, off, offc, ptr(dout), ptr(rowptr),
-                                                            ptr(edges), ptr(dY), ptr(dmax), first, stream_of(dout)),
-                      "pdgn_window_gather_sum_backward_csr")
-                first = 0
-                if hb == 2 and offc >= 0:
-                    dbias.append(group_colsum(dY.view(b * n, ldy)[:, offc:offc + C], n))
-                else:
-                    dbias.append(_dbias(dout, hb))
-            if dmax is not None:
-                mark_maxima(dY, dmax)
-            return (dY, None, None) + tuple(dbias)
-        dY = torch.zeros((b, n, ldy), dtype=F32, device=idx.device)
-        for (T, P, C, off, offc), dout, hb in zip(ctx.specs, douts, ctx.has_bias):
+        dY, dbias = _gather_sum_backward(idx, ctx.shape, ctx.specs, douts, ctx.has_bias)
+        return (dY, None, None) + tuple(dbias)
+
+
+def _gather_sum_forward(Y, idx, specs, biases):
+    b, n, ldy = Y.shape
+    k = idx.shape[2]
+    outs, partials = [], []
+    L = _lib.lib()
+    for spec, bias in zip(specs, biases):
+        T, P, C, off, offc = spec[:5]
+        out = torch.empty((b, n, P, C), dtype=F32, device=Y.device)
+        bias_c, bstride = _bias_arg(bias, C)
+        if len(spec) > 5 and spec[5]:
+            scr = torch.empty(L.pdgn_bn_scratch_floats(b * n * P, C), dtype=F32, device=Y.device)
+            check(L.pdgn_window_gather_sum_stats(b, n, k, ldy, T, P, C, off, offc, ptr(Y), ptr(idx), ptr(bias_c),
+                                                 bstride, ptr(out), ptr(scr), stream_of(Y)),
+                  "pdgn_window_gather_sum_stats")
+            partials.append(scr)
+        else:
+            check(L.pdgn_window_gather_sum(b, n, k, ldy, T, P, C, off, offc, ptr(Y), ptr(idx),
+                                           ptr(bias_c), bstride, ptr(out), stream_of(Y)),
+                  "pdgn_window_gather_sum")
+        outs.append(out)
+    return outs, partials
+
+
+def _gather_sum_backward(idx, shape, specs, douts, has_bias):
+    b, n, ldy, k = shape
+    douts = [d if d is not None else torch.zeros((b, n, P, C), dtype=F32, device=idx.device)
+             for d, (T, P, C, off, offc) in zip(douts, specs)]
+    L = _lib.lib()
+    covered = sum(T * C + (C if offc >= 0 else 0) for (T, P, C, off, offc) in specs)
+    vec_ok = ldy % 4 == 0 and k <= 31 and all(C % 4 == 0 and off % 4 == 0 and (offc < 0 or offc % 4 == 0)
+                                             for (T, P, C, off, offc) in specs)
+    dbias = []
+    if vec_ok and covered == ldy:
+        rowptr, edges = transposed_graph(idx)
+        dY = torch.empty((b, n, ldy), dtype=F32, device=idx.device)
+        dmax = row_maxima_buffer(b * n, idx.device) if (_lib.gemm_mode() == "x2" and b * n * ldy >= (1 << 24)) else None
+        first = 1
+        for (T, P, C, off, offc), dout, hb in zip(specs, douts, has_bias):
             hb = 3 if hb == 1 and has_zero_colsum(dout) else hb
             dout = dout.contiguous()
-            check(L.pdgn_window_gather_sum_backward(b, n, k, ldy, T, P, C, off, offc, ptr(dout), ptr(idx), ptr(dY),
-                                                    stream_of(dout)), "pdgn_window_gather_sum_backward")
-            dbias.append(_dbias(dout, hb))
-        return (dY, None, None) + tuple(dbias)
+            check(L.pdgn_window_gather_sum_backward_csr(b, n, k, ldy, T, P, C, off, offc, ptr(dout), ptr(rowptr),
+                                                        ptr(edges), ptr(dY), ptr(dmax), first, stream_of(dout)),
+                  "pdgn_window_gather_sum_backward_csr")
+            first = 0
+            if hb == 2 and offc >= 0:
+                dbias.append(group_colsum(dY.view(b * n, ldy)[:, offc:offc + C], n))
+            else:
+                dbias.append(_dbias(dout, hb))
+        if dmax is not None:
+            mark_maxima(dY, dmax)
+        return dY, dbias
+    dY = torch.zeros((b, n, ldy), dtype=F32, device=idx.device)
+    for (T, P, C, off, offc), dout, hb in zip(specs, douts, has_bias):
+        hb = 3 if hb == 1 and has_zero_colsum(dout) else hb
+        dout = dout.contiguous()
+        check(L.pdgn_window_gather_sum_backward(b, n, k, ldy, T, P, C, off, offc, ptr(dout), ptr(idx), ptr(dY),
+                                                stream_of(dout)), "pdgn_window_gather_sum_backward")
+        dbias.append(_dbias(dout, hb))
+    return dY, dbias
+
+
+def pair_gather_ok(Y, Yx, spec, spec_x, bias, bias_x):
+    if spec[:3] != spec_x[:3] or spec[0] != 1 or spec[2] % 4:
+        return False
+    for t, sp, bias_ in ((Y, spec, bias), (Yx, spec_x, bias_x)):
+        bc, bs = _bias_arg(bias_, sp[2]) if bias_ is not None else (None, 0)
+        if t.shape[2] % 4 or sp[3] % 4 or (sp[4] >= 0 and sp[4] % 4) or t.data_ptr() % 16 or not t.is_contiguous():
+            return False
+        if bc is not None and (bs % 4 or bc.data_ptr() % 16):
+            return False
+    return Y.shape[0] * Y.shape[1] * 31 < 2 ** 31
+
+
+class EdgeGatherSumPair(Function):
+
+    @staticmethod
+    def forward(ctx, Y, Yx, idx, specs, spec_x, bias_x, *biases):
+        require(Y, "Y", F32, 3)
+        require(Yx, "Yx", F32, 3)
+        require(idx, "idx", I32, 3)
+        b, n, ldy = Y.shape
+        k = idx.shape[2]
+        L = _lib.lib()
+        outs, partials = _gather_sum_forward(Y, idx, specs[:-1], biases[:-1])
+        T, P, C, off, offc = specs[-1][:5]
+        Tx, Px, Cx, offx, offcx = spec_x[:5]
+        if (T, P, C) != (Tx, Px, Cx):
+            raise ValueError("EdgeGatherSumPair: the paired specs differ in (T, P, C): %r / %r" % (specs[-1], spec_x))
+        out_a = torch.empty((b, n, P, C), dtype=F32, device=Y.device)
+        out_b = torch.empty((b, n, P, C), dtype=F32, device=Y.device)
+        parts = torch.empty((2, L.pdgn_bn_scratch_floats(b * n * P, C)), dtype=F32, device=Y.device)
+        ba, bsa = _bias_arg(biases[-1], C)
+        bx, bsx = _bias_arg(bias_x, C)
+        check(L.pdgn_pair_gather_stats(b, n, k, T, P, C, ptr(Y), ldy, off, offc, ptr(Yx), Yx.shape[2], offx, offcx, ptr(idx),
+                                       ptr(ba), bsa, ptr(bx), bsx, ptr(out_a), ptr(out_b), ptr(parts[0]), ptr(parts[1]), stream_of(Y)),
+              "pdgn_pair_gather_stats")
+        part_a, part_b = parts[0], parts[1]
+        ctx.mark_non_differentiable(*partials, part_a, part_b)
+        ctx.set_materialize_grads(False)
+        ctx.specs = tuple(tuple(spec[:5]) for spec in specs)
+        ctx.spec_x = tuple(spec_x[:5])
+        ctx.shape, ctx.shape_x = (b, n, ldy, k), (b, n, Yx.shape[2], k)
+        ctx.has_bias = [0 if bias is None else bias.dim() for bias in biases]
+        ctx.has_bias_x = 0 if bias_x is None else bias_x.dim()
+        ctx.save_for_backward(idx)
+        return tuple(outs) + (out_a, out_b) + tuple(partials) + (part_a, part_b)
+
+    @staticmethod
+    def backward(ctx, *douts):
+        (idx,) = ctx.saved_tensors
+        ns = len(ctx.specs)
+        dY, dbias = _gather_sum_backward(idx, ctx.shape, ctx.specs, douts[:ns], ctx.has_bias)
+        dYx, dbias_x = _gather_sum_backward(idx, ctx.shape_x, (ctx.spec_x,), douts[ns:ns + 1], [ctx.has_bias_x])
+        return (dY, dYx, None, None, None, dbias_x[0]) + tuple(dbias)
 
 
 def _dbias(dout, kind):
@@ -306,7 +376,8 @@
         return Wcat, Wb, T, P
 
     def _weights_key(self, Fc):
-        ws = [self.inte_conv_hk[0].weight, self.conv2.conv.weight] + ([self.conv_fea[0].weight, self.conv_all[3].weight] if self.bilateral else [])
+        ws = [self.inte_conv_hk[0].weight, self.conv2.conv.weight] + ([self.conv_fea[0].weight, self.conv_all[3].weight, self.conv_xyz[0].weight]
+                                                                      if self.bilateral else [])
         return (Fc, getattr(self, "_rows_hint", None)) + tuple((w.data_ptr(), w._version) for w in ws)
 
     def _assemble_now(self, Fc):
@@ -323,7 +394,8 @@
                    if self.bilateral and _lib.gemm_mode() == "x2" else None)
             if pa3 is not None and pa3.parts_p != 2:
                 pa3 = None
-        return WcatC, WcatV, Wb, pv, pb, pa3
+        Wxt = _XyzTaps.apply(_w2d(self.conv_xyz[0])) if self.bilateral else None
+        return WcatC, WcatV, Wb, pv, pb, pa3, Wxt
 
     def preassemble(self, Fc):
         self._pre = (self._weights_key(Fc), torch.is_grad_enabled(), self._assemble_now(Fc))
@@ -348,6 +420,11 @@
         if pre is not None and pre[0] == self._weights_key(Fc) and (pre[1] or not torch.is_grad_enabled()):
             return pre[2]
         return self._assemble_now(Fc)
+
+    def _xyz_product(self, pct, B, N, Wxt=None):
+        if Wxt is None:
+            Wxt = _XyzTaps.apply(_w2d(self.conv_xyz[0]))
+        return linear_cl(pct.reshape(B * N, 3), Wxt).view(B, N, -1)
 
     def forward(self, x, pc=None, idx=None):
         out = self.forward_cl(x.transpose(1, 2).contiguous(),
@@ -367,11 +444,11 @@
         elif idx.dtype != I32:
             idx = idx.to(I32)
         idx = idx.contiguous()
-        planes_v = planes_b = planes_a3 = None
+        planes_v = planes_b = planes_a3 = Wxt = None
         if xt.is_cuda:
             T = k // 2 + 1
             P = k - T + 1
-            WcatC, WcatV, Wb, planes_v, planes_b, planes_a3 = self.assembled(Fc if const is not None else 0)
+            WcatC, WcatV, Wb, planes_v, planes_b, planes_a3, Wxt = self.assembled(Fc if const is not None else 0)
         else:
             Wcat, Wb, T, P = self._assemble()
             WcatC, WcatV = (Wcat[:, :Fc], Wcat[:, Fc:].contiguous()) if const is not None else (None, Wcat)
@@ -398,17 +475,28 @@
         if knn_side is not None:
             torch.cuda.current_stream(idx.device).wait_event(knn_side)
             idx.record_stream(torch.cuda.current_stream(idx.device))
-        outs = EdgeGatherSum.apply(Y, idx, tuple(specs), *biases)
+        spec_x, Yx, paired = (1, k, 16, 0, 16), None, False
+        if self.bilateral and branch_pair_route(training, xt.is_cuda, 16):
+            Yx = self._xyz_product(pct, B, N, Wxt)
+            paired = pair_gather_ok(Y, Yx, specs[2], spec_x, biases[2], self.conv_xyz[0].bias)
+        if paired:
+            outs = EdgeGatherSumPair.apply(Y, Yx, idx, tuple(specs), spec_x, self.conv_xyz[0].bias, *biases)
+            part_i = outs[4] if fuse_stats else None
+        else:
+            outs = EdgeGatherSum.apply(Y, idx, tuple(specs), *biases)
+            part_i = outs[-1] if fuse_stats else None
         inte_pre, a_pre = outs[0], outs[1]
-        part_i = outs[-1] if fuse_stats else None
         w = None
         inte_max = inte_cmax = None
         if self.bilateral:
-            Wx = _w2d(self.conv_xyz[0])
-            Yx = linear_cl(pct.reshape(B * N, 3), _XyzTaps.apply(Wx)).view(B, N, -1)
-            (xyz_pre,) = EdgeGatherSum.apply(Yx, idx, ((1, k, 16, 0, 16),), self.conv_xyz[0].bias)
-            xyzf = bn_act(xyz_pre.view(-1, 16), self.conv_xyz[1], training)
-            h = bn_act(outs[2].view(-1, 16), self.conv_fea[1], training, mul=xyzf)
+            if paired:
+                h = bn_act_pair(outs[2].view(-1, 16), self.conv_fea[1], outs[-2], outs[3].view(-1, 16), self.conv_xyz[1], outs[-1])
+            else:
+                if Yx is None:
+                    Yx = self._xyz_product(pct, B, N, Wxt)
+                (xyz_pre,) = EdgeGatherSum.apply(Yx, idx, (spec_x,), self.conv_xyz[0].bias)
+                xyzf = bn_act(xyz_pre.view(-1, 16), self.conv_xyz[1], training)
+                h = bn_act(outs[2].view(-1, 16), self.conv_fea[1], training, mul=xyzf)
             h, ph = linear_cl(h, _w2d(self.conv_all[0]), None, None, training)
             h = bn_act(h, self.conv_all[1], training, pre_bias=self.conv_all[0].bias, partials=ph)
             h, ph = linear_cl(h, _w2d(self.conv_all[3]), None, None, training, planes=planes_a3)
diff --git a/pdgn_amd/fused.py b/pdgn_amd/fused.py
--- a/pdgn_amd/fused.py
+++ b/pdgn_amd/fused.py
@@ -216,6 +216,63 @@
             mark_zero_colsum(dx)
         return (dx, bs[C:], bs[:C], None, None, None, None, None, None, dmul, _pre_bias_grad(ctx.has_pre_bias, C, x.device),
                 None, None)
+
+
+_BRANCH_PAIR = [os.environ.get("PDGN_BRANCH_PAIR", "1") == "1"]
+
+
+def set_branch_pair(on):
+    old, _BRANCH_PAIR[0] = _BRANCH_PAIR[0], bool(on)
+    return old
+
+
+def branch_pair_route(training, is_cuda, C, bilateral=True):
+    return bool(_BRANCH_PAIR[0] and training and is_cuda and bilateral and C >= 4 and C % 4 == 0 and not _NO_FOLD)
+
+
+class BNActPair(Function):
+
+    @staticmethod
+    def forward(ctx, xa, xb, part_a, part_b, gamma_a, beta_a, rm_a, rv_a, momentum_a, eps_a, gamma_b, beta_b, rm_b, rv_b,
+                momentum_b, eps_b, act):
+        rows, C = xa.shape
+        xa, xb = xa.contiguous(), xb.contiguous()
+        L = _lib.lib()
+        ga, ba, gb, bb = (t.detach().contiguous() for t in (gamma_a, beta_a, gamma_b, beta_b))
+        stats = torch.empty((2, 4 * C), dtype=F32, device=xa.device)
+        check(L.pdgn_bn_pair_stats(rows, C, eps_a, momentum_a, ptr(ga), ptr(ba), None, ptr(rm_a), ptr(rv_a), ptr(part_a), ptr(xa), ptr(stats[0]),
+                                   eps_b, momentum_b, ptr(gb), ptr(bb), None, ptr(rm_b), ptr(rv_b), ptr(part_b), ptr(xb), ptr(stats[1]),
+                                   stream_of(xa)), "pdgn_bn_pair_stats")
+        h = torch.empty_like(xa)
+        check(L.pdgn_bn_act_pair_forward(rows, C, act, ptr(xa), ptr(stats[0]), ptr(xb), ptr(stats[1]), ptr(h), stream_of(xa)),
+              "pdgn_bn_act_pair_forward")
+        ctx.save_for_backward(xa, xb, stats)
+        ctx.cfg = (rows, C, act)
+        return h
+
+    @staticmethod
+    def backward(ctx, dh):
+        xa, xb, stats = ctx.saved_tensors
+        rows, C, act = ctx.cfg
+        dh = dh.contiguous()
+        L = _lib.lib()
+        scratch = torch.empty((2, _scratch_floats(L, rows, C)), dtype=F32, device=xa.device)
+        bs = torch.empty((2, 2 * C), dtype=F32, device=xa.device)
+        dxa, dxb = torch.empty_like(xa), torch.empty_like(xb)
+        check(L.pdgn_bn_act_pair_backward(rows, C, act, 1, ptr(xa), ptr(xb), ptr(dh), ptr(stats[0]), ptr(stats[1]), ptr(scratch[0]),
+                                          ptr(scratch[1]), ptr(bs[0]), ptr(bs[1]), ptr(dxa), ptr(dxb), stream_of(xa)),
+              "pdgn_bn_act_pair_backward")
+        mark_zero_colsum(dxa)
+        mark_zero_colsum(dxb)
+        return (dxa, dxb, None, None, bs[0, C:], bs[0, :C], None, None, None, None, bs[1, C:], bs[1, :C], None, None, None, None, None)
+
+
+def bn_act_pair(xa, bn_a, part_a, xb, bn_b, part_b, act="leaky_relu"):
+    for bn in (bn_a, bn_b):
+        if bn.track_running_stats:
+            _PENDING_COUNTS[bn.num_batches_tracked] = _PENDING_COUNTS.get(bn.num_batches_tracked, 0) + 1
+    return BNActPair.apply(xa, xb, part_a, part_b, bn_a.weight, bn_a.bias, bn_a.running_mean, bn_a.running_var, bn_a.momentum, bn_a.eps,
+                           bn_b.weight, bn_b.bias, bn_b.running_mean, bn_b.running_var, bn_b.momentum, bn_b.eps, ACT[act])
 
 
 _PENDING_COUNTS = {}
```

Result: no change. 3.139 million points/s (median of 4 runs) (+0.6%).
